# feng-li/dlsa

Hardware: AMD Instinct MI355X
Metric: rows/sec through X'WX kernel at p=500 (higher is better)
Workload: dtype f64

## Files before the change

### dlsa_amd/csrc/gram_cyclic.hip

```cpp
#include "common.h"
#ifndef DLSA_CYC_SPLIT
#define DLSA_CYC_SPLIT 1
#endif
#include <algorithm>
#ifndef DLSA_CYC_FLAGS
#define DLSA_CYC_FLAGS 0
#endif
#ifndef DLSA_CYC_PAIR
#define DLSA_CYC_PAIR 0
#endif
#ifndef DLSA_CYC_PRIO
#define DLSA_CYC_PRIO 0
#endif

namespace dlsa {

template <typename T>
void gram_reduce_launch(const T* partial, int nslab, int PP, int p, T* H, int64_t ldh, int accumulate, hipStream_t stream);

constexpr int CYC_NT = 31;
constexpr int CYC_C0 = 16 * CYC_NT;
constexpr int CYC_KC = 8;
constexpr int CYC_NST = 4;
constexpr int CYC_LDP = 528;
constexpr int CYC_BUF = CYC_KC * CYC_LDP + CYC_KC;
constexpr int CYC_GROUP = 4;
constexpr int CYC_PP = 512;
constexpr int CYC_MIN_P = 481, CYC_MAX_P = 508;
constexpr int64_t CYC_MIN_ROWS = 65536;

struct CycArgs {
    const double* X;
    const double* w;
    double* partial;
    int64_t ldx, n, rows_per_slab;
    int p;
    int nslab;
    unsigned long long* clk;
};

#include "gram_cyclic_asm.inc"

template <int T, int TEND, typename F>
__device__ __forceinline__ void cyc_for_tiles(F&& fn) {
    if constexpr (T < TEND) {
        double v[4];
        cyc_tile_read<T>(v);
        fn(T, v);
        cyc_for_tiles<T + 1, TEND>(fn);
    }
}

template <int K, int KEND, typename F>
__device__ __forceinline__ void cyc_for_tails(F&& fn) {
    if constexpr (K < KEND) {
        fn(K, cyc_tail_read<K>());
        cyc_for_tails<K + 1, KEND>(fn);
    }
}

template <bool HASW, int G>
__global__ __launch_bounds__(512, 2) void gram_cyclic_kernel(CycArgs a) {
    typedef __attribute__((address_space(3))) void* lds_ptr_t;
    constexpr int KC = CYC_KC, LDP = CYC_LDP, BUF = CYC_BUF, GA = G > 0 ? G : 1;
    constexpr int RW = 2, NW = 8, NB = RW + 7;
    constexpr int PIECES = KC * 4 / NW;
    constexpr int PPR = PIECES / RW;
    constexpr int DMA_PER_CHUNK = PIECES + (HASW ? 1 : 0);
    static_assert(KC == 8 && PPR * RW == PIECES && CYC_NST == 4, "pipeline shape");
    static_assert((BUF + 4 * LDP) * 8 + 128 < 65536, "stage parity + k-step offsets must fit a ds_read immediate");
    extern __shared__ __attribute__((aligned(16))) double lds[];
    const int tid = threadIdx.x, lane = tid & 63;
    const int wave = __builtin_amdgcn_readfirstlane(tid >> 6);
    const bool probe = blockIdx.x == 0 && wave == 0;
    const unsigned long long t_begin = probe ? __builtin_readcyclecounter() : 0ull;
    const int b = blockIdx.x, xcd = b % kNumXCD, jb = b / kNumXCD;
    const int slab = (jb / CYC_GROUP) * kNumXCD + xcd, member = jb % CYC_GROUP;
    const int rb = member * 4 + (wave & 3), db = wave >> 2;
    const int i0 = RW * rb, d0 = 8 * db;
    const bool two_rows = rb != 15;
    const bool tails = G > 0 && db == 0;

    const int64_t rbeg = (int64_t)slab * a.rows_per_slab;
    const int64_t rend = min(rbeg + a.rows_per_slab, a.n);
    const int64_t nrows = rend > rbeg ? rend - rbeg : 0;
    const int nchunks = (int)((nrows + KC - 1) / KC);

    const unsigned xbytes = nrows > 0 ? (unsigned)(((nrows - 1) * a.ldx + a.p) * 8) : 0u;
    __amdgpu_buffer_rsrc_t rsrcX = __builtin_amdgcn_make_buffer_rsrc((void*)(a.X + rbeg * a.ldx), 0, (int)xbytes, 0x00020000);
    __amdgpu_buffer_rsrc_t rsrcW =
        __builtin_amdgcn_make_buffer_rsrc((void*)(HASW ? a.w + rbeg : a.X), 0, HASW ? (int)(nrows * 8) : 0, 0x00020000);

    auto dma_piece = [&](int chunk, int buf, int pc) {
        const int id = pc * NW + wave, row = id >> 2, q = id & 3;
        const int soff = (int)((((int64_t)chunk * KC + row) * a.ldx + 128 * q) * 8);
        __builtin_amdgcn_raw_ptr_buffer_load_lds(rsrcX, (lds_ptr_t)(lds + buf * BUF + row * LDP + 128 * q), 16, lane * 16, soff, 0, 0);
    };
    auto dma_w = [&](int chunk, int buf) {
        if (HASW && lane < KC / 2)
            __builtin_amdgcn_raw_ptr_buffer_load_lds(rsrcW, (lds_ptr_t)(lds + buf * BUF + KC * LDP), 16, lane * 16, chunk * KC * 8, 0, 0);
    };

    cyc_acc_zero<128>();
    if constexpr (G > 0) cyc_tail_zero<2 * RW * G>();

#pragma unroll
    for (int ch = 0; ch < (DLSA_CYC_PAIR ? 2 : 3); ++ch) {
#pragma unroll
        for (int pc = 0; pc < PIECES; ++pc) dma_piece(ch, ch, pc);
        dma_w(ch, ch);
    }
#if DLSA_CYC_FLAGS
    unsigned long long* const flagL = reinterpret_cast<unsigned long long*>(lds + CYC_NST * BUF);
    unsigned long long* const flagD = flagL + 4;
    if (tid < 8) flagL[tid] = 0ull;
    __syncthreads();
    auto tag_of = [](int c) { return (unsigned)(((c >> 2) + 1) & 255); };
    auto post = [&](unsigned long long* f, int stage, int c) {
        if (lane == 0) reinterpret_cast<volatile unsigned char*>(f + stage)[wave] = (unsigned char)tag_of(c);
    };
    auto await = [&](unsigned long long* f, int stage, int c) {
        const unsigned long long want = 0x0101010101010101ull * tag_of(c);
        while (__builtin_amdgcn_readfirstlane((int)(*reinterpret_cast<volatile unsigned long long*>(f + stage) != want)))
            __builtin_amdgcn_s_sleep(1);
    };
    asm volatile("s_waitcnt vmcnt(%0)" ::"n"(2 * DMA_PER_CHUNK) : "memory");
    post(flagL, 0, 0);
    await(flagL, 0, 0);
#else
    asm volatile("s_waitcnt vmcnt(%0)" ::"n"(DLSA_CYC_PAIR ? 0 : 2 * DMA_PER_CHUNK) : "memory");
    asm volatile("s_barrier" ::: "memory");
#endif

    const int lane_part = ((lane >> 4) * LDP + (lane & 15)) * 8;
    int adA[2][RW], adB[2][NB], adT[2], adW[2];
#pragma unroll
    for (int sp = 0; sp < 2; ++sp) {
        const int sb = sp * 2 * BUF * 8;
        adA[sp][0] = sb + lane_part + 128 * i0;
        adA[sp][1] = sb + lane_part + 128 * (i0 + 1);
#pragma unroll
        for (int j = 0; j < NB; ++j) adB[sp][j] = sb + lane_part + 128 * ((i0 + d0 + j) % CYC_NT);
        adT[sp] = sb + ((lane >> 4) * LDP + CYC_C0 + (lane & 3)) * 8;
        adW[sp] = sb + (KC * LDP + (lane >> 4)) * 8;
    }
    const char* ldsb = (const char*)lds;
    struct Frag { double fa[RW], fb[NB], bt[GA], wv; };
    auto ld = [&](int addr, int imm) { return *(const double*)(ldsb + addr + imm); };
    auto load_frags = [&](int ST, int ks, Frag& f) {
        const int sp = ST >> 1, imm = ((ST & 1) * BUF + ks * 4 * LDP) * 8;
#pragma unroll
        for (int r = 0; r < RW; ++r) f.fa[r] = ld(adA[sp][r], imm);
#pragma unroll
        for (int j = 0; j < NB; ++j) f.fb[j] = ld(adB[sp][j], imm);
        if (tails) {
#pragma unroll
            for (int g = 0; g < G; ++g) f.bt[g] = ld(adT[sp], imm + 32 * g);
        }
        f.wv = HASW ? ld(adW[sp], ((ST & 1) * BUF + ks * 4) * 8) : 1.0;
    };
    auto kstep = [&](const Frag& f, int chunk_dma, int buf_dma, bool issue) {
        double aw[RW];
#pragma unroll
        for (int r = 0; r < RW; ++r) aw[r] = HASW ? f.fa[r] * f.wv : f.fa[r];
        cyc_row<0>(aw[0], f.fb[0], f.fb[1], f.fb[2], f.fb[3], f.fb[4], f.fb[5], f.fb[6], f.fb[7]);
        if (issue) {
#pragma unroll
            for (int k = 0; k < PPR; ++k) dma_piece(chunk_dma, buf_dma, k);
        }
        if (G > 0 || two_rows)
            cyc_row<1>(aw[1], f.fb[1], f.fb[2], f.fb[3], f.fb[4], f.fb[5], f.fb[6], f.fb[7], f.fb[8]);
        if (issue) {
#pragma unroll
            for (int k = 0; k < PPR; ++k) dma_piece(chunk_dma, buf_dma, PPR + k);
            dma_w(chunk_dma, buf_dma);
        }
        if constexpr (G > 0) {
            if (tails) cyc_tail_a<RW, G>(aw, f.bt);
        }
    };

    Frag fr0, fr1;
    load_frags(0, 0, fr0);
    if (DLSA_CYC_PRIO == 1 && db) __builtin_amdgcn_s_setprio(1);
    if (DLSA_CYC_PRIO == 2 && !db) __builtin_amdgcn_s_setprio(1);
#if DLSA_CYC_FLAGS
    for (int c4 = 0; c4 < nchunks; c4 += 4) {
#pragma unroll
        for (int u = 0; u < 4; ++u) {
            const int c = c4 + u;
            load_frags(u, 1, fr1);
            if (c > 0) post(flagD, (u + 3) & 3, c - 1);
            __builtin_amdgcn_sched_barrier(0);
            {
                double aw[RW];
#pragma unroll
                for (int r = 0; r < RW; ++r) aw[r] = HASW ? fr0.fa[r] * fr0.wv : fr0.fa[r];
                cyc_row<0>(aw[0], fr0.fb[0], fr0.fb[1], fr0.fb[2], fr0.fb[3], fr0.fb[4], fr0.fb[5], fr0.fb[6], fr0.fb[7]);
                __builtin_amdgcn_sched_barrier(0);
                asm volatile("s_waitcnt vmcnt(%0)" ::"n"(DMA_PER_CHUNK) : "memory");
                post(flagL, (u + 1) & 3, c + 1);
                __builtin_amdgcn_sched_barrier(0);
                if (G > 0 || two_rows)
                    cyc_row<1>(aw[1], fr0.fb[1], fr0.fb[2], fr0.fb[3], fr0.fb[4], fr0.fb[5], fr0.fb[6], fr0.fb[7], fr0.fb[8]);
                if constexpr (G > 0) {
                    if (tails) cyc_tail_a<RW, G>(aw, fr0.bt);
                }
                __builtin_amdgcn_sched_barrier(0);
            }
            await(flagL, (u + 1) & 3, c + 1);
            load_frags((u + 1) & 3, 0, fr0);
            __builtin_amdgcn_sched_barrier(0);
            if (c > 0) await(flagD, (u + 3) & 3, c - 1);
            __builtin_amdgcn_sched_barrier(0);
            kstep(fr1, c + 3, (u + 3) & 3, true);
            __builtin_amdgcn_sched_barrier(0);
        }
    }
#elif DLSA_CYC_PAIR
    for (int c4 = 0; c4 < nchunks; c4 += 4) {
#pragma unroll
        for (int u = 0; u < 4; u += 2) {
            const int c = c4 + u;
            load_frags(u, 1, fr1);
            __builtin_amdgcn_sched_barrier(0);
            kstep(fr0, c + 2, (u + 2) & 3, true);
            __builtin_amdgcn_sched_barrier(0);
            load_frags(u + 1, 0, fr0);
            __builtin_amdgcn_sched_barrier(0);
            kstep(fr1, c + 3, (u + 3) & 3, true);
            __builtin_amdgcn_sched_barrier(0);
            load_frags(u + 1, 1, fr1);
            __builtin_amdgcn_sched_barrier(0);
            kstep(fr0, 0, 0, false);
            __builtin_amdgcn_sched_barrier(0);
            {
                double aw[RW];
#pragma unroll
                for (int r = 0; r < RW; ++r) aw[r] = HASW ? fr1.fa[r] * fr1.wv : fr1.fa[r];
                cyc_row<0>(aw[0], fr1.fb[0], fr1.fb[1], fr1.fb[2], fr1.fb[3], fr1.fb[4], fr1.fb[5], fr1.fb[6], fr1.fb[7]);
                __builtin_amdgcn_sched_barrier(0);
                if (db) {
                    asm volatile("s_waitcnt vmcnt(0)" ::: "memory");
                    asm volatile("s_barrier" ::: "memory");
                }
                if (G > 0 || two_rows)
                    cyc_row<1>(aw[1], fr1.fb[1], fr1.fb[2], fr1.fb[3], fr1.fb[4], fr1.fb[5], fr1.fb[6], fr1.fb[7], fr1.fb[8]);
                if constexpr (G > 0) {
                    if (tails) cyc_tail_a<RW, G>(aw, fr1.bt);
                }
                __builtin_amdgcn_sched_barrier(0);
                if (!db) {
                    asm volatile("s_waitcnt vmcnt(0)" ::: "memory");
                    asm volatile("s_barrier" ::: "memory");
                }
            }
            load_frags((u + 2) & 3, 0, fr0);
            __builtin_amdgcn_sched_barrier(0);
        }
    }
#else
    for (int c4 = 0; c4 < nchunks; c4 += 4) {
#pragma unroll
        for (int u = 0; u < 4; ++u) {
            load_frags(u, 1, fr1);
            __builtin_amdgcn_sched_barrier(0);
#if DLSA_CYC_SPLIT
            {
                double aw[RW];
#pragma unroll
                for (int r = 0; r < RW; ++r) aw[r] = HASW ? fr0.fa[r] * fr0.wv : fr0.fa[r];
                cyc_row<0>(aw[0], fr0.fb[0], fr0.fb[1], fr0.fb[2], fr0.fb[3], fr0.fb[4], fr0.fb[5], fr0.fb[6], fr0.fb[7]);
                __builtin_amdgcn_sched_barrier(0);
                if (db) {
                    asm volatile("s_waitcnt vmcnt(%0)" ::"n"(DMA_PER_CHUNK) : "memory");
                    asm volatile("s_barrier" ::: "memory");
                }
                if (G > 0 || two_rows)
                    cyc_row<1>(aw[1], fr0.fb[1], fr0.fb[2], fr0.fb[3], fr0.fb[4], fr0.fb[5], fr0.fb[6], fr0.fb[7], fr0.fb[8]);
                if constexpr (G > 0) {
                    if (tails) cyc_tail_a<RW, G>(aw, fr0.bt);
                }
                __builtin_amdgcn_sched_barrier(0);
                if (!db) {
                    asm volatile("s_waitcnt vmcnt(%0)" ::"n"(DMA_PER_CHUNK) : "memory");
                    asm volatile("s_barrier" ::: "memory");
                }
            }
#else
            kstep(fr0, 0, 0, false);
            __builtin_amdgcn_sched_barrier(0);
            asm volatile("s_waitcnt vmcnt(%0)" ::"n"(DMA_PER_CHUNK) : "memory");
            asm volatile("s_barrier" ::: "memory");
#endif
            load_frags((u + 1) & 3, 0, fr0);
            __builtin_amdgcn_sched_barrier(0);
            kstep(fr1, c4 + u + 3, (u + 3) & 3, true);
            __builtin_amdgcn_sched_barrier(0);
        }
    }
#endif
    asm volatile("s_waitcnt vmcnt(0)" ::: "memory");
    asm volatile("s_nop 15\n\ts_nop 15" ::: "memory");

    double* __restrict__ P = a.partial + (int64_t)slab * CYC_PP * CYC_PP;
    const int nt_rows = two_rows ? 2 : 1;
    cyc_for_tiles<0, 8 * RW>([&](int k, double (&v)[4]) {
        const int r = k >> 3, cdist = k & 7;
        if (r < nt_rows) {
            const int it = i0 + r, jt = (it + d0 + cdist) % CYC_NT;
#pragma unroll
            for (int q = 0; q < 4; ++q) {
                const int rr = 16 * it + 4 * q + (lane >> 4), cc = 16 * jt + (lane & 15);
                if (jt >= it) P[(int64_t)rr * CYC_PP + cc] = v[q];
                else P[(int64_t)cc * CYC_PP + rr] = v[q];
            }
        }
    });
    if constexpr (G > 0) {
        if (tails) cyc_for_tails<0, RW * G>([&](int idx, double v) {
            const int s = idx / G, g = idx - s * G;
            const int row = 16 * (i0 + s) + 4 * ((lane & 15) >> 2) + (lane >> 4), col = CYC_C0 + 4 * g + (lane & 3);
            P[(int64_t)row * CYC_PP + col] = v;
        });
    }
    if (probe && lane == 0) *a.clk = __builtin_readcyclecounter() - t_begin;
}

static int cyc_slabs(int64_t n, int64_t& rows_per_slab) {
    int64_t ns = kNumCU / CYC_GROUP;
    while (ns > kNumXCD && n / ns < 4 * CYC_KC) ns -= kNumXCD;
    rows_per_slab = ((n + ns - 1) / ns + CYC_KC - 1) / CYC_KC * CYC_KC;
    return (int)ns;
}

bool gram_cyclic_shape_ok(int64_t n, int p) { return p >= CYC_MIN_P && p <= CYC_MAX_P && n >= CYC_MIN_ROWS; }

bool gram_cyclic_eligible(const double* X, int64_t ldx, const double* w, int64_t n, int p) {
    if (!gram_cyclic_shape_ok(n, p)) return false;
    if (gram_dbg_env() & 8) return false;
    int64_t rps;
    cyc_slabs(n, rps);
    return ldx % 2 == 0 && ((uintptr_t)X % 16) == 0 && (!w || ((uintptr_t)w % 16) == 0) &&
           (double)(rps + 8 * CYC_KC) * (double)ldx * 8.0 < 2.0e9;
}

size_t gram_cyclic_ws_bytes(int64_t n, int p) {
    int64_t rps;
    return align_up((size_t)cyc_slabs(n, rps) * CYC_PP * CYC_PP * 8, 256) + kGramProbeBytes;
}

int gram_cyclic_f64(const double* X, int64_t ldx, const double* w, int64_t n, int p, double* H, int64_t ldh,
                    int accumulate, void* ws, size_t ws_bytes, hipStream_t stream) {
    CycArgs a;
    a.X = X; a.w = w; a.partial = (double*)ws; a.ldx = ldx; a.n = n;
    a.p = p + (p & 1);
    a.nslab = cyc_slabs(n, a.rows_per_slab);
    const size_t need = align_up((size_t)a.nslab * CYC_PP * CYC_PP * 8, 256) + kGramProbeBytes;
    a.clk = (unsigned long long*)((char*)ws + need - kGramProbeBytes);
    if (!ws || ws_bytes < need || ((uintptr_t)ws & 255)) {
        set_error("gram: workspace %zu bytes needed (256-aligned), got %zu", need, ws_bytes);
        return DLSA_ERR_WORKSPACE;
    }
    const int g = a.p <= CYC_C0 ? 0 : (a.p - CYC_C0 + 3) / 4;
    const size_t shm = (size_t)CYC_NST * CYC_BUF * 8 + (DLSA_CYC_FLAGS ? 64 : 0);
    const int blocks = a.nslab * CYC_GROUP;
#define DLSA_LAUNCH_CYC(HW, GV) do { \
        DLSA_HIP_CHECK(hipFuncSetAttribute(reinterpret_cast<const void*>(gram_cyclic_kernel<HW, GV>), \
                                           hipFuncAttributeMaxDynamicSharedMemorySize, (int)shm)); \
        hipLaunchKernelGGL((gram_cyclic_kernel<HW, GV>), dim3(blocks), dim3(512), shm, stream, a); } while (0)
#define DLSA_LAUNCH_CYC_G(HW) do { switch (g) { \
        case 0: DLSA_LAUNCH_CYC(HW, 0); break; case 1: DLSA_LAUNCH_CYC(HW, 1); break; \
        case 2: DLSA_LAUNCH_CYC(HW, 2); break; default: DLSA_LAUNCH_CYC(HW, 3); break; } } while (0)
    if (w) DLSA_LAUNCH_CYC_G(true);
    else DLSA_LAUNCH_CYC_G(false);
    note_gram_kernel(a.clk, stream, "gram_cyclic_kernel<%s,%d>", w ? "true" : "false", g > 3 ? 3 : g);
#undef DLSA_LAUNCH_CYC_G
#undef DLSA_LAUNCH_CYC
    DLSA_HIP_CHECK(hipGetLastError());
    gram_reduce_launch<double>((const double*)ws, a.nslab, CYC_PP, p, H, ldh, accumulate, stream);
    DLSA_HIP_CHECK(hipGetLastError());
    return DLSA_OK;
}

}
```

### dlsa_amd/csrc/gram_cyclic_asm.inc

```
template <int NREG> __device__ __forceinline__ void cyc_acc_zero();
template <> __device__ __forceinline__ void cyc_acc_zero<128>() {
    asm volatile("v_accvgpr_write_b32 a0, 0\n\tv_accvgpr_write_b32 a1, 0\n\tv_accvgpr_write_b32 a2, 0\n\tv_accvgpr_write_b32 a3, 0\n\tv_accvgpr_write_b32 a4, 0\n\tv_accvgpr_write_b32 a5, 0\n\tv_accvgpr_write_b32 a6, 0\n\tv_accvgpr_write_b32 a7, 0\n\tv_accvgpr_write_b32 a8, 0\n\tv_accvgpr_write_b32 a9, 0\n\tv_accvgpr_write_b32 a10, 0\n\tv_accvgpr_write_b32 a11, 0\n\tv_accvgpr_write_b32 a12, 0\n\tv_accvgpr_write_b32 a13, 0\n\tv_accvgpr_write_b32 a14, 0\n\tv_accvgpr_write_b32 a15, 0\n\tv_accvgpr_write_b32 a16, 0\n\tv_accvgpr_write_b32 a17, 0\n\tv_accvgpr_write_b32 a18, 0\n\tv_accvgpr_write_b32 a19, 0\n\tv_accvgpr_write_b32 a20, 0\n\tv_accvgpr_write_b32 a21, 0\n\tv_accvgpr_write_b32 a22, 0\n\tv_accvgpr_write_b32 a23, 0\n\tv_accvgpr_write_b32 a24, 0\n\tv_accvgpr_write_b32 a25, 0\n\tv_accvgpr_write_b32 a26, 0\n\tv_accvgpr_write_b32 a27, 0\n\tv_accvgpr_write_b32 a28, 0\n\tv_accvgpr_write_b32 a29, 0\n\tv_accvgpr_write_b32 a30, 0\n\tv_accvgpr_write_b32 a31, 0\n\tv_accvgpr_write_b32 a32, 0\n\tv_accvgpr_write_b32 a33, 0\n\tv_accvgpr_write_b32 a34, 0\n\tv_accvgpr_write_b32 a35, 0\n\tv_accvgpr_write_b32 a36, 0\n\tv_accvgpr_write_b32 a37, 0\n\tv_accvgpr_write_b32 a38, 0\n\tv_accvgpr_write_b32 a39, 0\n\tv_accvgpr_write_b32 a40, 0\n\tv_accvgpr_write_b32 a41, 0\n\tv_accvgpr_write_b32 a42, 0\n\tv_accvgpr_write_b32 a43, 0\n\tv_accvgpr_write_b32 a44, 0\n\tv_accvgpr_write_b32 a45, 0\n\tv_accvgpr_write_b32 a46, 0\n\tv_accvgpr_write_b32 a47, 0\n\tv_accvgpr_write_b32 a48, 0\n\tv_accvgpr_write_b32 a49, 0\n\tv_accvgpr_write_b32 a50, 0\n\tv_accvgpr_write_b32 a51, 0\n\tv_accvgpr_write_b32 a52, 0\n\tv_accvgpr_write_b32 a53, 0\n\tv_accvgpr_write_b32 a54, 0\n\tv_accvgpr_write_b32 a55, 0\n\tv_accvgpr_write_b32 a56, 0\n\tv_accvgpr_write_b32 a57, 0\n\tv_accvgpr_write_b32 a58, 0\n\tv_accvgpr_write_b32 a59, 0\n\tv_accvgpr_write_b32 a60, 0\n\tv_accvgpr_write_b32 a61, 0\n\tv_accvgpr_write_b32 a62, 0\n\tv_accvgpr_write_b32 a63, 0\n\tv_accvgpr_write_b32 a64, 0\n\tv_accvgpr_write_b32 a65, 0\n\tv_accvgpr_write_b32 a66, 0\n\tv_accvgpr_write_b32 a67, 0\n\tv_accvgpr_write_b32 a68, 0\n\tv_accvgpr_write_b32 a69, 0\n\tv_accvgpr_write_b32 a70, 0\n\tv_accvgpr_write_b32 a71, 0\n\tv_accvgpr_write_b32 a72, 0\n\tv_accvgpr_write_b32 a73, 0\n\tv_accvgpr_write_b32 a74, 0\n\tv_accvgpr_write_b32 a75, 0\n\tv_accvgpr_write_b32 a76, 0\n\tv_accvgpr_write_b32 a77, 0\n\tv_accvgpr_write_b32 a78, 0\n\tv_accvgpr_write_b32 a79, 0\n\tv_accvgpr_write_b32 a80, 0\n\tv_accvgpr_write_b32 a81, 0\n\tv_accvgpr_write_b32 a82, 0\n\tv_accvgpr_write_b32 a83, 0\n\tv_accvgpr_write_b32 a84, 0\n\tv_accvgpr_write_b32 a85, 0\n\tv_accvgpr_write_b32 a86, 0\n\tv_accvgpr_write_b32 a87, 0\n\tv_accvgpr_write_b32 a88, 0\n\tv_accvgpr_write_b32 a89, 0\n\tv_accvgpr_write_b32 a90, 0\n\tv_accvgpr_write_b32 a91, 0\n\tv_accvgpr_write_b32 a92, 0\n\tv_accvgpr_write_b32 a93, 0\n\tv_accvgpr_write_b32 a94, 0\n\tv_accvgpr_write_b32 a95, 0\n\tv_accvgpr_write_b32 a96, 0\n\tv_accvgpr_write_b32 a97, 0\n\tv_accvgpr_write_b32 a98, 0\n\tv_accvgpr_write_b32 a99, 0\n\tv_accvgpr_write_b32 a100, 0\n\tv_accvgpr_write_b32 a101, 0\n\tv_accvgpr_write_b32 a102, 0\n\tv_accvgpr_write_b32 a103, 0\n\tv_accvgpr_write_b32 a104, 0\n\tv_accvgpr_write_b32 a105, 0\n\tv_accvgpr_write_b32 a106, 0\n\tv_accvgpr_write_b32 a107, 0\n\tv_accvgpr_write_b32 a108, 0\n\tv_accvgpr_write_b32 a109, 0\n\tv_accvgpr_write_b32 a110, 0\n\tv_accvgpr_write_b32 a111, 0\n\tv_accvgpr_write_b32 a112, 0\n\tv_accvgpr_write_b32 a113, 0\n\tv_accvgpr_write_b32 a114, 0\n\tv_accvgpr_write_b32 a115, 0\n\tv_accvgpr_write_b32 a116, 0\n\tv_accvgpr_write_b32 a117, 0\n\tv_accvgpr_write_b32 a118, 0\n\tv_accvgpr_write_b32 a119, 0\n\tv_accvgpr_write_b32 a120, 0\n\tv_accvgpr_write_b32 a121, 0\n\tv_accvgpr_write_b32 a122, 0\n\tv_accvgpr_write_b32 a123, 0\n\tv_accvgpr_write_b32 a124, 0\n\tv_accvgpr_write_b32 a125, 0\n\tv_accvgpr_write_b32 a126, 0\n\tv_accvgpr_write_b32 a127, 0" ::: "a0", "a1", "a2", "a3", "a4", "a5", "a6", "a7", "a8", "a9", "a10", "a11", "a12", "a13", "a14", "a15", "a16", "a17", "a18", "a19", "a20", "a21", "a22", "a23", "a24", "a25", "a26", "a27", "a28", "a29", "a30", "a31", "a32", "a33", "a34", "a35", "a36", "a37", "a38", "a39", "a40", "a41", "a42", "a43", "a44", "a45", "a46", "a47", "a48", "a49", "a50", "a51", "a52", "a53", "a54", "a55", "a56", "a57", "a58", "a59", "a60", "a61", "a62", "a63", "a64", "a65", "a66", "a67", "a68", "a69", "a70", "a71", "a72", "a73", "a74", "a75", "a76", "a77", "a78", "a79", "a80", "a81", "a82", "a83", "a84", "a85", "a86", "a87", "a88", "a89", "a90", "a91", "a92", "a93", "a94", "a95", "a96", "a97", "a98", "a99", "a100", "a101", "a102", "a103", "a104", "a105", "a106", "a107", "a108", "a109", "a110", "a111", "a112", "a113", "a114", "a115", "a116", "a117", "a118", "a119", "a120", "a121", "a122", "a123", "a124", "a125", "a126", "a127");
}
template <> __device__ __forceinline__ void cyc_acc_zero<256>() {
    asm volatile("v_accvgpr_write_b32 a0, 0\n\tv_accvgpr_write_b32 a1, 0\n\tv_accvgpr_write_b32 a2, 0\n\tv_accvgpr_write_b32 a3, 0\n\tv_accvgpr_write_b32 a4, 0\n\tv_accvgpr_write_b32 a5, 0\n\tv_accvgpr_write_b32 a6, 0\n\tv_accvgpr_write_b32 a7, 0\n\tv_accvgpr_write_b32 a8, 0\n\tv_accvgpr_write_b32 a9, 0\n\tv_accvgpr_write_b32 a10, 0\n\tv_accvgpr_write_b32 a11, 0\n\tv_accvgpr_write_b32 a12, 0\n\tv_accvgpr_write_b32 a13, 0\n\tv_accvgpr_write_b32 a14, 0\n\tv_accvgpr_write_b32 a15, 0\n\tv_accvgpr_write_b32 a16, 0\n\tv_accvgpr_write_b32 a17, 0\n\tv_accvgpr_write_b32 a18, 0\n\tv_accvgpr_write_b32 a19, 0\n\tv_accvgpr_write_b32 a20, 0\n\tv_accvgpr_write_b32 a21, 0\n\tv_accvgpr_write_b32 a22, 0\n\tv_accvgpr_write_b32 a23, 0\n\tv_accvgpr_write_b32 a24, 0\n\tv_accvgpr_write_b32 a25, 0\n\tv_accvgpr_write_b32 a26, 0\n\tv_accvgpr_write_b32 a27, 0\n\tv_accvgpr_write_b32 a28, 0\n\tv_accvgpr_write_b32 a29, 0\n\tv_accvgpr_write_b32 a30, 0\n\tv_accvgpr_write_b32 a31, 0\n\tv_accvgpr_write_b32 a32, 0\n\tv_accvgpr_write_b32 a33, 0\n\tv_accvgpr_write_b32 a34, 0\n\tv_accvgpr_write_b32 a35, 0\n\tv_accvgpr_write_b32 a36, 0\n\tv_accvgpr_write_b32 a37, 0\n\tv_accvgpr_write_b32 a38, 0\n\tv_accvgpr_write_b32 a39, 0\n\tv_accvgpr_write_b32 a40, 0\n\tv_accvgpr_write_b32 a41, 0\n\tv_accvgpr_write_b32 a42, 0\n\tv_accvgpr_write_b32 a43, 0\n\tv_accvgpr_write_b32 a44, 0\n\tv_accvgpr_write_b32 a45, 0\n\tv_accvgpr_write_b32 a46, 0\n\tv_accvgpr_write_b32 a47, 0\n\tv_accvgpr_write_b32 a48, 0\n\tv_accvgpr_write_b32 a49, 0\n\tv_accvgpr_write_b32 a50, 0\n\tv_accvgpr_write_b32 a51, 0\n\tv_accvgpr_write_b32 a52, 0\n\tv_accvgpr_write_b32 a53, 0\n\tv_accvgpr_write_b32 a54, 0\n\tv_accvgpr_write_b32 a55, 0\n\tv_accvgpr_write_b32 a56, 0\n\tv_accvgpr_write_b32 a57, 0\n\tv_accvgpr_write_b32 a58, 0\n\tv_accvgpr_write_b32 a59, 0\n\tv_accvgpr_write_b32 a60, 0\n\tv_accvgpr_write_b32 a61, 0\n\tv_accvgpr_write_b32 a62, 0\n\tv_accvgpr_write_b32 a63, 0\n\tv_accvgpr_write_b32 a64, 0\n\tv_accvgpr_write_b32 a65, 0\n\tv_accvgpr_write_b32 a66, 0\n\tv_accvgpr_write_b32 a67, 0\n\tv_accvgpr_write_b32 a68, 0\n\tv_accvgpr_write_b32 a69, 0\n\tv_accvgpr_write_b32 a70, 0\n\tv_accvgpr_write_b32 a71, 0\n\tv_accvgpr_write_b32 a72, 0\n\tv_accvgpr_write_b32 a73, 0\n\tv_accvgpr_write_b32 a74, 0\n\tv_accvgpr_write_b32 a75, 0\n\tv_accvgpr_write_b32 a76, 0\n\tv_accvgpr_write_b32 a77, 0\n\tv_accvgpr_write_b32 a78, 0\n\tv_accvgpr_write_b32 a79, 0\n\tv_accvgpr_write_b32 a80, 0\n\tv_accvgpr_write_b32 a81, 0\n\tv_accvgpr_write_b32 a82, 0\n\tv_accvgpr_write_b32 a83, 0\n\tv_accvgpr_write_b32 a84, 0\n\tv_accvgpr_write_b32 a85, 0\n\tv_accvgpr_write_b32 a86, 0\n\tv_accvgpr_write_b32 a87, 0\n\tv_accvgpr_write_b32 a88, 0\n\tv_accvgpr_write_b32 a89, 0\n\tv_accvgpr_write_b32 a90, 0\n\tv_accvgpr_write_b32 a91, 0\n\tv_accvgpr_write_b32 a92, 0\n\tv_accvgpr_write_b32 a93, 0\n\tv_accvgpr_write_b32 a94, 0\n\tv_accvgpr_write_b32 a95, 0\n\tv_accvgpr_write_b32 a96, 0\n\tv_accvgpr_write_b32 a97, 0\n\tv_accvgpr_write_b32 a98, 0\n\tv_accvgpr_write_b32 a99, 0\n\tv_accvgpr_write_b32 a100, 0\n\tv_accvgpr_write_b32 a101, 0\n\tv_accvgpr_write_b32 a102, 0\n\tv_accvgpr_write_b32 a103, 0\n\tv_accvgpr_write_b32 a104, 0\n\tv_accvgpr_write_b32 a105, 0\n\tv_accvgpr_write_b32 a106, 0\n\tv_accvgpr_write_b32 a107, 0\n\tv_accvgpr_write_b32 a108, 0\n\tv_accvgpr_write_b32 a109, 0\n\tv_accvgpr_write_b32 a110, 0\n\tv_accvgpr_write_b32 a111, 0\n\tv_accvgpr_write_b32 a112, 0\n\tv_accvgpr_write_b32 a113, 0\n\tv_accvgpr_write_b32 a114, 0\n\tv_accvgpr_write_b32 a115, 0\n\tv_accvgpr_write_b32 a116, 0\n\tv_accvgpr_write_b32 a117, 0\n\tv_accvgpr_write_b32 a118, 0\n\tv_accvgpr_write_b32 a119, 0\n\tv_accvgpr_write_b32 a120, 0\n\tv_accvgpr_write_b32 a121, 0\n\tv_accvgpr_write_b32 a122, 0\n\tv_accvgpr_write_b32 a123, 0\n\tv_accvgpr_write_b32 a124, 0\n\tv_accvgpr_write_b32 a125, 0\n\tv_accvgpr_write_b32 a126, 0\n\tv_accvgpr_write_b32 a127, 0\n\tv_accvgpr_write_b32 a128, 0\n\tv_accvgpr_write_b32 a129, 0\n\tv_accvgpr_write_b32 a130, 0\n\tv_accvgpr_write_b32 a131, 0\n\tv_accvgpr_write_b32 a132, 0\n\tv_accvgpr_write_b32 a133, 0\n\tv_accvgpr_write_b32 a134, 0\n\tv_accvgpr_write_b32 a135, 0\n\tv_accvgpr_write_b32 a136, 0\n\tv_accvgpr_write_b32 a137, 0\n\tv_accvgpr_write_b32 a138, 0\n\tv_accvgpr_write_b32 a139, 0\n\tv_accvgpr_write_b32 a140, 0\n\tv_accvgpr_write_b32 a141, 0\n\tv_accvgpr_write_b32 a142, 0\n\tv_accvgpr_write_b32 a143, 0\n\tv_accvgpr_write_b32 a144, 0\n\tv_accvgpr_write_b32 a145, 0\n\tv_accvgpr_write_b32 a146, 0\n\tv_accvgpr_write_b32 a147, 0\n\tv_accvgpr_write_b32 a148, 0\n\tv_accvgpr_write_b32 a149, 0\n\tv_accvgpr_write_b32 a150, 0\n\tv_accvgpr_write_b32 a151, 0\n\tv_accvgpr_write_b32 a152, 0\n\tv_accvgpr_write_b32 a153, 0\n\tv_accvgpr_write_b32 a154, 0\n\tv_accvgpr_write_b32 a155, 0\n\tv_accvgpr_write_b32 a156, 0\n\tv_accvgpr_write_b32 a157, 0\n\tv_accvgpr_write_b32 a158, 0\n\tv_accvgpr_write_b32 a159, 0\n\tv_accvgpr_write_b32 a160, 0\n\tv_accvgpr_write_b32 a161, 0\n\tv_accvgpr_write_b32 a162, 0\n\tv_accvgpr_write_b32 a163, 0\n\tv_accvgpr_write_b32 a164, 0\n\tv_accvgpr_write_b32 a165, 0\n\tv_accvgpr_write_b32 a166, 0\n\tv_accvgpr_write_b32 a167, 0\n\tv_accvgpr_write_b32 a168, 0\n\tv_accvgpr_write_b32 a169, 0\n\tv_accvgpr_write_b32 a170, 0\n\tv_accvgpr_write_b32 a171, 0\n\tv_accvgpr_write_b32 a172, 0\n\tv_accvgpr_write_b32 a173, 0\n\tv_accvgpr_write_b32 a174, 0\n\tv_accvgpr_write_b32 a175, 0\n\tv_accvgpr_write_b32 a176, 0\n\tv_accvgpr_write_b32 a177, 0\n\tv_accvgpr_write_b32 a178, 0\n\tv_accvgpr_write_b32 a179, 0\n\tv_accvgpr_write_b32 a180, 0\n\tv_accvgpr_write_b32 a181, 0\n\tv_accvgpr_write_b32 a182, 0\n\tv_accvgpr_write_b32 a183, 0\n\tv_accvgpr_write_b32 a184, 0\n\tv_accvgpr_write_b32 a185, 0\n\tv_accvgpr_write_b32 a186, 0\n\tv_accvgpr_write_b32 a187, 0\n\tv_accvgpr_write_b32 a188, 0\n\tv_accvgpr_write_b32 a189, 0\n\tv_accvgpr_write_b32 a190, 0\n\tv_accvgpr_write_b32 a191, 0\n\tv_accvgpr_write_b32 a192, 0\n\tv_accvgpr_write_b32 a193, 0\n\tv_accvgpr_write_b32 a194, 0\n\tv_accvgpr_write_b32 a195, 0\n\tv_accvgpr_write_b32 a196, 0\n\tv_accvgpr_write_b32 a197, 0\n\tv_accvgpr_write_b32 a198, 0\n\tv_accvgpr_write_b32 a199, 0\n\tv_accvgpr_write_b32 a200, 0\n\tv_accvgpr_write_b32 a201, 0\n\tv_accvgpr_write_b32 a202, 0\n\tv_accvgpr_write_b32 a203, 0\n\tv_accvgpr_write_b32 a204, 0\n\tv_accvgpr_write_b32 a205, 0\n\tv_accvgpr_write_b32 a206, 0\n\tv_accvgpr_write_b32 a207, 0\n\tv_accvgpr_write_b32 a208, 0\n\tv_accvgpr_write_b32 a209, 0\n\tv_accvgpr_write_b32 a210, 0\n\tv_accvgpr_write_b32 a211, 0\n\tv_accvgpr_write_b32 a212, 0\n\tv_accvgpr_write_b32 a213, 0\n\tv_accvgpr_write_b32 a214, 0\n\tv_accvgpr_write_b32 a215, 0\n\tv_accvgpr_write_b32 a216, 0\n\tv_accvgpr_write_b32 a217, 0\n\tv_accvgpr_write_b32 a218, 0\n\tv_accvgpr_write_b32 a219, 0\n\tv_accvgpr_write_b32 a220, 0\n\tv_accvgpr_write_b32 a221, 0\n\tv_accvgpr_write_b32 a222, 0\n\tv_accvgpr_write_b32 a223, 0\n\tv_accvgpr_write_b32 a224, 0\n\tv_accvgpr_write_b32 a225, 0\n\tv_accvgpr_write_b32 a226, 0\n\tv_accvgpr_write_b32 a227, 0\n\tv_accvgpr_write_b32 a228, 0\n\tv_accvgpr_write_b32 a229, 0\n\tv_accvgpr_write_b32 a230, 0\n\tv_accvgpr_write_b32 a231, 0\n\tv_accvgpr_write_b32 a232, 0\n\tv_accvgpr_write_b32 a233, 0\n\tv_accvgpr_write_b32 a234, 0\n\tv_accvgpr_write_b32 a235, 0\n\tv_accvgpr_write_b32 a236, 0\n\tv_accvgpr_write_b32 a237, 0\n\tv_accvgpr_write_b32 a238, 0\n\tv_accvgpr_write_b32 a239, 0\n\tv_accvgpr_write_b32 a240, 0\n\tv_accvgpr_write_b32 a241, 0\n\tv_accvgpr_write_b32 a242, 0\n\tv_accvgpr_write_b32 a243, 0\n\tv_accvgpr_write_b32 a244, 0\n\tv_accvgpr_write_b32 a245, 0\n\tv_accvgpr_write_b32 a246, 0\n\tv_accvgpr_write_b32 a247, 0\n\tv_accvgpr_write_b32 a248, 0\n\tv_accvgpr_write_b32 a249, 0\n\tv_accvgpr_write_b32 a250, 0\n\tv_accvgpr_write_b32 a251, 0\n\tv_accvgpr_write_b32 a252, 0\n\tv_accvgpr_write_b32 a253, 0\n\tv_accvgpr_write_b32 a254, 0\n\tv_accvgpr_write_b32 a255, 0" ::: "a0", "a1", "a2", "a3", "a4", "a5", "a6", "a7", "a8", "a9", "a10", "a11", "a12", "a13", "a14", "a15", "a16", "a17", "a18", "a19", "a20", "a21", "a22", "a23", "a24", "a25", "a26", "a27", "a28", "a29", "a30", "a31", "a32", "a33", "a34", "a35", "a36", "a37", "a38", "a39", "a40", "a41", "a42", "a43", "a44", "a45", "a46", "a47", "a48", "a49", "a50", "a51", "a52", "a53", "a54", "a55", "a56", "a57", "a58", "a59", "a60", "a61", "a62", "a63", "a64", "a65", "a66", "a67", "a68", "a69", "a70", "a71", "a72", "a73", "a74", "a75", "a76", "a77", "a78", "a79", "a80", "a81", "a82", "a83", "a84", "a85", "a86", "a87", "a88", "a89", "a90", "a91", "a92", "a93", "a94", "a95", "a96", "a97", "a98", "a99", "a100", "a101", "a102", "a103", "a104", "a105", "a106", "a107", "a108", "a109", "a110", "a111", "a112", "a113", "a114", "a115", "a116", "a117", "a118", "a119", "a120", "a121", "a122", "a123", "a124", "a125", "a126", "a127", "a128", "a129", "a130", "a131", "a132", "a133", "a134", "a135", "a136", "a137", "a138", "a139", "a140", "a141", "a142", "a143", "a144", "a145", "a146", "a147", "a148", "a149", "a150", "a151", "a152", "a153", "a154", "a155", "a156", "a157", "a158", "a159", "a160", "a161", "a162", "a163", "a164", "a165", "a166", "a167", "a168", "a169", "a170", "a171", "a172", "a173", "a174", "a175", "a176", "a177", "a178", "a179", "a180", "a181", "a182", "a183", "a184", "a185", "a186", "a187", "a188", "a189", "a190", "a191", "a192", "a193", "a194", "a195", "a196", "a197", "a198", "a199", "a200", "a201", "a202", "a203", "a204", "a205", "a206", "a207", "a208", "a209", "a210", "a211", "a212", "a213", "a214", "a215", "a216", "a217", "a218", "a219", "a220", "a221", "a222", "a223", "a224", "a225", "a226", "a227", "a228", "a229", "a230", "a231", "a232", "a233", "a234", "a235", "a236", "a237", "a238", "a239", "a240", "a241", "a242", "a243", "a244", "a245", "a246", "a247", "a248", "a249", "a250", "a251", "a252", "a253", "a254", "a255");
}
template <int R> __device__ __forceinline__ void cyc_row(double a, double b0, double b1, double b2, double b3, double b4, double b5, double b6, double b7);
template <> __device__ __forceinline__ void cyc_row<0>(double a, double b0, double b1, double b2, double b3, double b4, double b5, double b6, double b7) {
    asm volatile("s_nop 1\n\tv_mfma_f64_16x16x4_f64 a[0:7], %0, %1, a[0:7]\n\tv_mfma_f64_16x16x4_f64 a[8:15], %0, %2, a[8:15]\n\tv_mfma_f64_16x16x4_f64 a[16:23], %0, %3, a[16:23]\n\tv_mfma_f64_16x16x4_f64 a[24:31], %0, %4, a[24:31]\n\tv_mfma_f64_16x16x4_f64 a[32:39], %0, %5, a[32:39]\n\tv_mfma_f64_16x16x4_f64 a[40:47], %0, %6, a[40:47]\n\tv_mfma_f64_16x16x4_f64 a[48:55], %0, %7, a[48:55]\n\tv_mfma_f64_16x16x4_f64 a[56:63], %0, %8, a[56:63]"
                 :: "v"(a), "v"(b0), "v"(b1), "v"(b2), "v"(b3), "v"(b4), "v"(b5), "v"(b6), "v"(b7)
                 : "a0", "a1", "a2", "a3", "a4", "a5", "a6", "a7", "a8", "a9", "a10", "a11", "a12", "a13", "a14", "a15", "a16", "a17", "a18", "a19", "a20", "a21", "a22", "a23", "a24", "a25", "a26", "a27", "a28", "a29", "a30", "a31", "a32", "a33", "a34", "a35", "a36", "a37", "a38", "a39", "a40", "a41", "a42", "a43", "a44", "a45", "a46", "a47", "a48", "a49", "a50", "a51", "a52", "a53", "a54", "a55", "a56", "a57", "a58", "a59", "a60", "a61", "a62", "a63");
}
template <> __device__ __forceinline__ void cyc_row<1>(double a, double b0, double b1, double b2, double b3, double b4, double b5, double b6, double b7) {
    asm volatile("s_nop 1\n\tv_mfma_f64_16x16x4_f64 a[64:71], %0, %1, a[64:71]\n\tv_mfma_f64_16x16x4_f64 a[72:79], %0, %2, a[72:79]\n\tv_mfma_f64_16x16x4_f64 a[80:87], %0, %3, a[80:87]\n\tv_mfma_f64_16x16x4_f64 a[88:95], %0, %4, a[88:95]\n\tv_mfma_f64_16x16x4_f64 a[96:103], %0, %5, a[96:103]\n\tv_mfma_f64_16x16x4_f64 a[104:111], %0, %6, a[104:111]\n\tv_mfma_f64_16x16x4_f64 a[112:119], %0, %7, a[112:119]\n\tv_mfma_f64_16x16x4_f64 a[120:127], %0, %8, a[120:127]"
                 :: "v"(a), "v"(b0), "v"(b1), "v"(b2), "v"(b3), "v"(b4), "v"(b5), "v"(b6), "v"(b7)
                 : "a64", "a65", "a66", "a67", "a68", "a69", "a70", "a71", "a72", "a73", "a74", "a75", "a76", "a77", "a78", "a79", "a80", "a81", "a82", "a83", "a84", "a85", "a86", "a87", "a88", "a89", "a90", "a91", "a92", "a93", "a94", "a95", "a96", "a97", "a98", "a99", "a100", "a101", "a102", "a103", "a104", "a105", "a106", "a107", "a108", "a109", "a110", "a111", "a112", "a113", "a114", "a115", "a116", "a117", "a118", "a119", "a120", "a121", "a122", "a123", "a124", "a125", "a126", "a127");
}
template <> __device__ __forceinline__ void cyc_row<2>(double a, double b0, double b1, double b2, double b3, double b4, double b5, double b6, double b7) {
    asm volatile("s_nop 1\n\tv_mfma_f64_16x16x4_f64 a[128:135], %0, %1, a[128:135]\n\tv_mfma_f64_16x16x4_f64 a[136:143], %0, %2, a[136:143]\n\tv_mfma_f64_16x16x4_f64 a[144:151], %0, %3, a[144:151]\n\tv_mfma_f64_16x16x4_f64 a[152:159], %0, %4, a[152:159]\n\tv_mfma_f64_16x16x4_f64 a[160:167], %0, %5, a[160:167]\n\tv_mfma_f64_16x16x4_f64 a[168:175], %0, %6, a[168:175]\n\tv_mfma_f64_16x16x4_f64 a[176:183], %0, %7, a[176:183]\n\tv_mfma_f64_16x16x4_f64 a[184:191], %0, %8, a[184:191]"
                 :: "v"(a), "v"(b0), "v"(b1), "v"(b2), "v"(b3), "v"(b4), "v"(b5), "v"(b6), "v"(b7)
                 : "a128", "a129", "a130", "a131", "a132", "a133", "a134", "a135", "a136", "a137", "a138", "a139", "a140", "a141", "a142", "a143", "a144", "a145", "a146", "a147", "a148", "a149", "a150", "a151", "a152", "a153", "a154", "a155", "a156", "a157", "a158", "a159", "a160", "a161", "a162", "a163", "a164", "a165", "a166", "a167", "a168", "a169", "a170", "a171", "a172", "a173", "a174", "a175", "a176", "a177", "a178", "a179", "a180", "a181", "a182", "a183", "a184", "a185", "a186", "a187", "a188", "a189", "a190", "a191");
}
template <> __device__ __forceinline__ void cyc_row<3>(double a, double b0, double b1, double b2, double b3, double b4, double b5, double b6, double b7) {
    asm volatile("s_nop 1\n\tv_mfma_f64_16x16x4_f64 a[192:199], %0, %1, a[192:199]\n\tv_mfma_f64_16x16x4_f64 a[200:207], %0, %2, a[200:207]\n\tv_mfma_f64_16x16x4_f64 a[208:215], %0, %3, a[208:215]\n\tv_mfma_f64_16x16x4_f64 a[216:223], %0, %4, a[216:223]\n\tv_mfma_f64_16x16x4_f64 a[224:231], %0, %5, a[224:231]\n\tv_mfma_f64_16x16x4_f64 a[232:239], %0, %6, a[232:239]\n\tv_mfma_f64_16x16x4_f64 a[240:247], %0, %7, a[240:247]\n\tv_mfma_f64_16x16x4_f64 a[248:255], %0, %8, a[248:255]"
                 :: "v"(a), "v"(b0), "v"(b1), "v"(b2), "v"(b3), "v"(b4), "v"(b5), "v"(b6), "v"(b7)
                 : "a192", "a193", "a194", "a195", "a196", "a197", "a198", "a199", "a200", "a201", "a202", "a203", "a204", "a205", "a206", "a207", "a208", "a209", "a210", "a211", "a212", "a213", "a214", "a215", "a216", "a217", "a218", "a219", "a220", "a221", "a222", "a223", "a224", "a225", "a226", "a227", "a228", "a229", "a230", "a231", "a232", "a233", "a234", "a235", "a236", "a237", "a238", "a239", "a240", "a241", "a242", "a243", "a244", "a245", "a246", "a247", "a248", "a249", "a250", "a251", "a252", "a253", "a254", "a255");
}
template <int TS, int G> __device__ __forceinline__ void cyc_tail_a(const double (&at)[TS], const double (&bt)[G > 0 ? G : 1]);
template <int N> __device__ __forceinline__ void cyc_tail_zero();
template <> __device__ __forceinline__ void cyc_tail_zero<4>() {
    asm volatile("v_accvgpr_write_b32 a128, 0\n\tv_accvgpr_write_b32 a129, 0\n\tv_accvgpr_write_b32 a130, 0\n\tv_accvgpr_write_b32 a131, 0" ::: "a128", "a129", "a130", "a131");
}
template <> __device__ __forceinline__ void cyc_tail_zero<8>() {
    asm volatile("v_accvgpr_write_b32 a128, 0\n\tv_accvgpr_write_b32 a129, 0\n\tv_accvgpr_write_b32 a130, 0\n\tv_accvgpr_write_b32 a131, 0\n\tv_accvgpr_write_b32 a132, 0\n\tv_accvgpr_write_b32 a133, 0\n\tv_accvgpr_write_b32 a134, 0\n\tv_accvgpr_write_b32 a135, 0" ::: "a128", "a129", "a130", "a131", "a132", "a133", "a134", "a135");
}
template <> __device__ __forceinline__ void cyc_tail_zero<12>() {
    asm volatile("v_accvgpr_write_b32 a128, 0\n\tv_accvgpr_write_b32 a129, 0\n\tv_accvgpr_write_b32 a130, 0\n\tv_accvgpr_write_b32 a131, 0\n\tv_accvgpr_write_b32 a132, 0\n\tv_accvgpr_write_b32 a133, 0\n\tv_accvgpr_write_b32 a134, 0\n\tv_accvgpr_write_b32 a135, 0\n\tv_accvgpr_write_b32 a136, 0\n\tv_accvgpr_write_b32 a137, 0\n\tv_accvgpr_write_b32 a138, 0\n\tv_accvgpr_write_b32 a139, 0" ::: "a128", "a129", "a130", "a131", "a132", "a133", "a134", "a135", "a136", "a137", "a138", "a139");
}
template <> __device__ __forceinline__ void cyc_tail_a<2, 0>(const double (&)[2], const double (&)[1]) {}
template <> __device__ __forceinline__ void cyc_tail_a<2, 1>(const double (&at)[2], const double (&bt)[1]) {
    asm volatile("v_mfma_f64_4x4x4_4b_f64 a[128:129], %0, %2, a[128:129]\n\tv_mfma_f64_4x4x4_4b_f64 a[130:131], %1, %2, a[130:131]"
                 :: "v"(at[0]), "v"(at[1]), "v"(bt[0])
                 : "a128", "a129", "a130", "a131");
}
template <> __device__ __forceinline__ void cyc_tail_a<2, 2>(const double (&at)[2], const double (&bt)[2]) {
    asm volatile("v_mfma_f64_4x4x4_4b_f64 a[128:129], %0, %2, a[128:129]\n\tv_mfma_f64_4x4x4_4b_f64 a[130:131], %0, %3, a[130:131]\n\tv_mfma_f64_4x4x4_4b_f64 a[132:133], %1, %2, a[132:133]\n\tv_mfma_f64_4x4x4_4b_f64 a[134:135], %1, %3, a[134:135]"
                 :: "v"(at[0]), "v"(at[1]), "v"(bt[0]), "v"(bt[1])
                 : "a128", "a129", "a130", "a131", "a132", "a133", "a134", "a135");
}
template <> __device__ __forceinline__ void cyc_tail_a<2, 3>(const double (&at)[2], const double (&bt)[3]) {
    asm volatile("v_mfma_f64_4x4x4_4b_f64 a[128:129], %0, %2, a[128:129]\n\tv_mfma_f64_4x4x4_4b_f64 a[130:131], %0, %3, a[130:131]\n\tv_mfma_f64_4x4x4_4b_f64 a[132:133], %0, %4, a[132:133]\n\tv_mfma_f64_4x4x4_4b_f64 a[134:135], %1, %2, a[134:135]\n\tv_mfma_f64_4x4x4_4b_f64 a[136:137], %1, %3, a[136:137]\n\tv_mfma_f64_4x4x4_4b_f64 a[138:139], %1, %4, a[138:139]"
                 :: "v"(at[0]), "v"(at[1]), "v"(bt[0]), "v"(bt[1]), "v"(bt[2])
                 : "a128", "a129", "a130", "a131", "a132", "a133", "a134", "a135", "a136", "a137", "a138", "a139");
}
template <int IDX> __device__ __forceinline__ double cyc_tail_read() {
    int lo, hi;
    if constexpr (IDX == 0) asm volatile("v_accvgpr_read_b32 %0, a128\n\tv_accvgpr_read_b32 %1, a129" : "=v"(lo), "=v"(hi));
    else if constexpr (IDX == 1) asm volatile("v_accvgpr_read_b32 %0, a130\n\tv_accvgpr_read_b32 %1, a131" : "=v"(lo), "=v"(hi));
    else if constexpr (IDX == 2) asm volatile("v_accvgpr_read_b32 %0, a132\n\tv_accvgpr_read_b32 %1, a133" : "=v"(lo), "=v"(hi));
    else if constexpr (IDX == 3) asm volatile("v_accvgpr_read_b32 %0, a134\n\tv_accvgpr_read_b32 %1, a135" : "=v"(lo), "=v"(hi));
    else if constexpr (IDX == 4) asm volatile("v_accvgpr_read_b32 %0, a136\n\tv_accvgpr_read_b32 %1, a137" : "=v"(lo), "=v"(hi));
    else if constexpr (IDX == 5) asm volatile("v_accvgpr_read_b32 %0, a138\n\tv_accvgpr_read_b32 %1, a139" : "=v"(lo), "=v"(hi));
    return __hiloint2double(hi, lo);
}
template <int T> __device__ __forceinline__ void cyc_tile_read(double (&v)[4]) {
    int w0, w1, w2, w3, w4, w5, w6, w7;
    if constexpr (T == 0) asm volatile("v_accvgpr_read_b32 %0, a0\n\tv_accvgpr_read_b32 %1, a1\n\tv_accvgpr_read_b32 %2, a2\n\tv_accvgpr_read_b32 %3, a3\n\tv_accvgpr_read_b32 %4, a4\n\tv_accvgpr_read_b32 %5, a5\n\tv_accvgpr_read_b32 %6, a6\n\tv_accvgpr_read_b32 %7, a7" : "=v"(w0), "=v"(w1), "=v"(w2), "=v"(w3), "=v"(w4), "=v"(w5), "=v"(w6), "=v"(w7));
    else if constexpr (T == 1) asm volatile("v_accvgpr_read_b32 %0, a8\n\tv_accvgpr_read_b32 %1, a9\n\tv_accvgpr_read_b32 %2, a10\n\tv_accvgpr_read_b32 %3, a11\n\tv_accvgpr_read_b32 %4, a12\n\tv_accvgpr_read_b32 %5, a13\n\tv_accvgpr_read_b32 %6, a14\n\tv_accvgpr_read_b32 %7, a15" : "=v"(w0), "=v"(w1), "=v"(w2), "=v"(w3), "=v"(w4), "=v"(w5), "=v"(w6), "=v"(w7));
    else if constexpr (T == 2) asm volatile("v_accvgpr_read_b32 %0, a16\n\tv_accvgpr_read_b32 %1, a17\n\tv_accvgpr_read_b32 %2, a18\n\tv_accvgpr_read_b32 %3, a19\n\tv_accvgpr_read_b32 %4, a20\n\tv_accvgpr_read_b32 %5, a21\n\tv_accvgpr_read_b32 %6, a22\n\tv_accvgpr_read_b32 %7, a23" : "=v"(w0), "=v"(w1), "=v"(w2), "=v"(w3), "=v"(w4), "=v"(w5), "=v"(w6), "=v"(w7));
    else if constexpr (T == 3) asm volatile("v_accvgpr_read_b32 %0, a24\n\tv_accvgpr_read_b32 %1, a25\n\tv_accvgpr_read_b32 %2, a26\n\tv_accvgpr_read_b32 %3, a27\n\tv_accvgpr_read_b32 %4, a28\n\tv_accvgpr_read_b32 %5, a29\n\tv_accvgpr_read_b32 %6, a30\n\tv_accvgpr_read_b32 %7, a31" : "=v"(w0), "=v"(w1), "=v"(w2), "=v"(w3), "=v"(w4), "=v"(w5), "=v"(w6), "=v"(w7));
    else if constexpr (T == 4) asm volatile("v_accvgpr_read_b32 %0, a32\n\tv_accvgpr_read_b32 %1, a33\n\tv_accvgpr_read_b32 %2, a34\n\tv_accvgpr_read_b32 %3, a35\n\tv_accvgpr_read_b32 %4, a36\n\tv_accvgpr_read_b32 %5, a37\n\tv_accvgpr_read_b32 %6, a38\n\tv_accvgpr_read_b32 %7, a39" : "=v"(w0), "=v"(w1), "=v"(w2), "=v"(w3), "=v"(w4), "=v"(w5), "=v"(w6), "=v"(w7));
    else if constexpr (T == 5) asm volatile("v_accvgpr_read_b32 %0, a40\n\tv_accvgpr_read_b32 %1, a41\n\tv_accvgpr_read_b32 %2, a42\n\tv_accvgpr_read_b32 %3, a43\n\tv_accvgpr_read_b32 %4, a44\n\tv_accvgpr_read_b32 %5, a45\n\tv_accvgpr_read_b32 %6, a46\n\tv_accvgpr_read_b32 %7, a47" : "=v"(w0), "=v"(w1), "=v"(w2), "=v"(w3), "=v"(w4), "=v"(w5), "=v"(w6), "=v"(w7));
    else if constexpr (T == 6) asm volatile("v_accvgpr_read_b32 %0, a48\n\tv_accvgpr_read_b32 %1, a49\n\tv_accvgpr_read_b32 %2, a50\n\tv_accvgpr_read_b32 %3, a51\n\tv_accvgpr_read_b32 %4, a52\n\tv_accvgpr_read_b32 %5, a53\n\tv_accvgpr_read_b32 %6, a54\n\tv_accvgpr_read_b32 %7, a55" : "=v"(w0), "=v"(w1), "=v"(w2), "=v"(w3), "=v"(w4), "=v"(w5), "=v"(w6), "=v"(w7));
    else if constexpr (T == 7) asm volatile("v_accvgpr_read_b32 %0, a56\n\tv_accvgpr_read_b32 %1, a57\n\tv_accvgpr_read_b32 %2, a58\n\tv_accvgpr_read_b32 %3, a59\n\tv_accvgpr_read_b32 %4, a60\n\tv_accvgpr_read_b32 %5, a61\n\tv_accvgpr_read_b32 %6, a62\n\tv_accvgpr_read_b32 %7, a63" : "=v"(w0), "=v"(w1), "=v"(w2), "=v"(w3), "=v"(w4), "=v"(w5), "=v"(w6), "=v"(w7));
    else if constexpr (T == 8) asm volatile("v_accvgpr_read_b32 %0, a64\n\tv_accvgpr_read_b32 %1, a65\n\tv_accvgpr_read_b32 %2, a66\n\tv_accvgpr_read_b32 %3, a67\n\tv_accvgpr_read_b32 %4, a68\n\tv_accvgpr_read_b32 %5, a69\n\tv_accvgpr_read_b32 %6, a70\n\tv_accvgpr_read_b32 %7, a71" : "=v"(w0), "=v"(w1), "=v"(w2), "=v"(w3), "=v"(w4), "=v"(w5), "=v"(w6), "=v"(w7));
    else if constexpr (T == 9) asm volatile("v_accvgpr_read_b32 %0, a72\n\tv_accvgpr_read_b32 %1, a73\n\tv_accvgpr_read_b32 %2, a74\n\tv_accvgpr_read_b32 %3, a75\n\tv_accvgpr_read_b32 %4, a76\n\tv_accvgpr_read_b32 %5, a77\n\tv_accvgpr_read_b32 %6, a78\n\tv_accvgpr_read_b32 %7, a79" : "=v"(w0), "=v"(w1), "=v"(w2), "=v"(w3), "=v"(w4), "=v"(w5), "=v"(w6), "=v"(w7));
    else if constexpr (T == 10) asm volatile("v_accvgpr_read_b32 %0, a80\n\tv_accvgpr_read_b32 %1, a81\n\tv_accvgpr_read_b32 %2, a82\n\tv_accvgpr_read_b32 %3, a83\n\tv_accvgpr_read_b32 %4, a84\n\tv_accvgpr_read_b32 %5, a85\n\tv_accvgpr_read_b32 %6, a86\n\tv_accvgpr_read_b32 %7, a87" : "=v"(w0), "=v"(w1), "=v"(w2), "=v"(w3), "=v"(w4), "=v"(w5), "=v"(w6), "=v"(w7));
    else if constexpr (T == 11) asm volatile("v_accvgpr_read_b32 %0, a88\n\tv_accvgpr_read_b32 %1, a89\n\tv_accvgpr_read_b32 %2, a90\n\tv_accvgpr_read_b32 %3, a91\n\tv_accvgpr_read_b32 %4, a92\n\tv_accvgpr_read_b32 %5, a93\n\tv_accvgpr_read_b32 %6, a94\n\tv_accvgpr_read_b32 %7, a95" : "=v"(w0), "=v"(w1), "=v"(w2), "=v"(w3), "=v"(w4), "=v"(w5), "=v"(w6), "=v"(w7));
    else if constexpr (T == 12) asm volatile("v_accvgpr_read_b32 %0, a96\n\tv_accvgpr_read_b32 %1, a97\n\tv_accvgpr_read_b32 %2, a98\n\tv_accvgpr_read_b32 %3, a99\n\tv_accvgpr_read_b32 %4, a100\n\tv_accvgpr_read_b32 %5, a101\n\tv_accvgpr_read_b32 %6, a102\n\tv_accvgpr_read_b32 %7, a103" : "=v"(w0), "=v"(w1), "=v"(w2), "=v"(w3), "=v"(w4), "=v"(w5), "=v"(w6), "=v"(w7));
    else if constexpr (T == 13) asm volatile("v_accvgpr_read_b32 %0, a104\n\tv_accvgpr_read_b32 %1, a105\n\tv_accvgpr_read_b32 %2, a106\n\tv_accvgpr_read_b32 %3, a107\n\tv_accvgpr_read_b32 %4, a108\n\tv_accvgpr_read_b32 %5, a109\n\tv_accvgpr_read_b32 %6, a110\n\tv_accvgpr_read_b32 %7, a111" : "=v"(w0), "=v"(w1), "=v"(w2), "=v"(w3), "=v"(w4), "=v"(w5), "=v"(w6), "=v"(w7));
    else if constexpr (T == 14) asm volatile("v_accvgpr_read_b32 %0, a112\n\tv_accvgpr_read_b32 %1, a113\n\tv_accvgpr_read_b32 %2, a114\n\tv_accvgpr_read_b32 %3, a115\n\tv_accvgpr_read_b32 %4, a116\n\tv_accvgpr_read_b32 %5, a117\n\tv_accvgpr_read_b32 %6, a118\n\tv_accvgpr_read_b32 %7, a119" : "=v"(w0), "=v"(w1), "=v"(w2), "=v"(w3), "=v"(w4), "=v"(w5), "=v"(w6), "=v"(w7));
    else if constexpr (T == 15) asm volatile("v_accvgpr_read_b32 %0, a120\n\tv_accvgpr_read_b32 %1, a121\n\tv_accvgpr_read_b32 %2, a122\n\tv_accvgpr_read_b32 %3, a123\n\tv_accvgpr_read_b32 %4, a124\n\tv_accvgpr_read_b32 %5, a125\n\tv_accvgpr_read_b32 %6, a126\n\tv_accvgpr_read_b32 %7, a127" : "=v"(w0), "=v"(w1), "=v"(w2), "=v"(w3), "=v"(w4), "=v"(w5), "=v"(w6), "=v"(w7));
    else if constexpr (T == 16) asm volatile("v_accvgpr_read_b32 %0, a128\n\tv_accvgpr_read_b32 %1, a129\n\tv_accvgpr_read_b32 %2, a130\n\tv_accvgpr_read_b32 %3, a131\n\tv_accvgpr_read_b32 %4, a132\n\tv_accvgpr_read_b32 %5, a133\n\tv_accvgpr_read_b32 %6, a134\n\tv_accvgpr_read_b32 %7, a135" : "=v"(w0), "=v"(w1), "=v"(w2), "=v"(w3), "=v"(w4), "=v"(w5), "=v"(w6), "=v"(w7));
    else if constexpr (T == 17) asm volatile("v_accvgpr_read_b32 %0, a136\n\tv_accvgpr_read_b32 %1, a137\n\tv_accvgpr_read_b32 %2, a138\n\tv_accvgpr_read_b32 %3, a139\n\tv_accvgpr_read_b32 %4, a140\n\tv_accvgpr_read_b32 %5, a141\n\tv_accvgpr_read_b32 %6, a142\n\tv_accvgpr_read_b32 %7, a143" : "=v"(w0), "=v"(w1), "=v"(w2), "=v"(w3), "=v"(w4), "=v"(w5), "=v"(w6), "=v"(w7));
    else if constexpr (T == 18) asm volatile("v_accvgpr_read_b32 %0, a144\n\tv_accvgpr_read_b32 %1, a145\n\tv_accvgpr_read_b32 %2, a146\n\tv_accvgpr_read_b32 %3, a147\n\tv_accvgpr_read_b32 %4, a148\n\tv_accvgpr_read_b32 %5, a149\n\tv_accvgpr_read_b32 %6, a150\n\tv_accvgpr_read_b32 %7, a151" : "=v"(w0), "=v"(w1), "=v"(w2), "=v"(w3), "=v"(w4), "=v"(w5), "=v"(w6), "=v"(w7));
    else if constexpr (T == 19) asm volatile("v_accvgpr_read_b32 %0, a152\n\tv_accvgpr_read_b32 %1, a153\n\tv_accvgpr_read_b32 %2, a154\n\tv_accvgpr_read_b32 %3, a155\n\tv_accvgpr_read_b32 %4, a156\n\tv_accvgpr_read_b32 %5, a157\n\tv_accvgpr_read_b32 %6, a158\n\tv_accvgpr_read_b32 %7, a159" : "=v"(w0), "=v"(w1), "=v"(w2), "=v"(w3), "=v"(w4), "=v"(w5), "=v"(w6), "=v"(w7));
    else if constexpr (T == 20) asm volatile("v_accvgpr_read_b32 %0, a160\n\tv_accvgpr_read_b32 %1, a161\n\tv_accvgpr_read_b32 %2, a162\n\tv_accvgpr_read_b32 %3, a163\n\tv_accvgpr_read_b32 %4, a164\n\tv_accvgpr_read_b32 %5, a165\n\tv_accvgpr_read_b32 %6, a166\n\tv_accvgpr_read_b32 %7, a167" : "=v"(w0), "=v"(w1), "=v"(w2), "=v"(w3), "=v"(w4), "=v"(w5), "=v"(w6), "=v"(w7));
    else if constexpr (T == 21) asm volatile("v_accvgpr_read_b32 %0, a168\n\tv_accvgpr_read_b32 %1, a169\n\tv_accvgpr_read_b32 %2, a170\n\tv_accvgpr_read_b32 %3, a171\n\tv_accvgpr_read_b32 %4, a172\n\tv_accvgpr_read_b32 %5, a173\n\tv_accvgpr_read_b32 %6, a174\n\tv_accvgpr_read_b32 %7, a175" : "=v"(w0), "=v"(w1), "=v"(w2), "=v"(w3), "=v"(w4), "=v"(w5), "=v"(w6), "=v"(w7));
    else if constexpr (T == 22) asm volatile("v_accvgpr_read_b32 %0, a176\n\tv_accvgpr_read_b32 %1, a177\n\tv_accvgpr_read_b32 %2, a178\n\tv_accvgpr_read_b32 %3, a179\n\tv_accvgpr_read_b32 %4, a180\n\tv_accvgpr_read_b32 %5, a181\n\tv_accvgpr_read_b32 %6, a182\n\tv_accvgpr_read_b32 %7, a183" : "=v"(w0), "=v"(w1), "=v"(w2), "=v"(w3), "=v"(w4), "=v"(w5), "=v"(w6), "=v"(w7));
    else if constexpr (T == 23) asm volatile("v_accvgpr_read_b32 %0, a184\n\tv_accvgpr_read_b32 %1, a185\n\tv_accvgpr_read_b32 %2, a186\n\tv_accvgpr_read_b32 %3, a187\n\tv_accvgpr_read_b32 %4, a188\n\tv_accvgpr_read_b32 %5, a189\n\tv_accvgpr_read_b32 %6, a190\n\tv_accvgpr_read_b32 %7, a191" : "=v"(w0), "=v"(w1), "=v"(w2), "=v"(w3), "=v"(w4), "=v"(w5), "=v"(w6), "=v"(w7));
    else if constexpr (T == 24) asm volatile("v_accvgpr_read_b32 %0, a192\n\tv_accvgpr_read_b32 %1, a193\n\tv_accvgpr_read_b32 %2, a194\n\tv_accvgpr_read_b32 %3, a195\n\tv_accvgpr_read_b32 %4, a196\n\tv_accvgpr_read_b32 %5, a197\n\tv_accvgpr_read_b32 %6, a198\n\tv_accvgpr_read_b32 %7, a199" : "=v"(w0), "=v"(w1), "=v"(w2), "=v"(w3), "=v"(w4), "=v"(w5), "=v"(w6), "=v"(w7));
    else if constexpr (T == 25) asm volatile("v_accvgpr_read_b32 %0, a200\n\tv_accvgpr_read_b32 %1, a201\n\tv_accvgpr_read_b32 %2, a202\n\tv_accvgpr_read_b32 %3, a203\n\tv_accvgpr_read_b32 %4, a204\n\tv_accvgpr_read_b32 %5, a205\n\tv_accvgpr_read_b32 %6, a206\n\tv_accvgpr_read_b32 %7, a207" : "=v"(w0), "=v"(w1), "=v"(w2), "=v"(w3), "=v"(w4), "=v"(w5), "=v"(w6), "=v"(w7));
    else if constexpr (T == 26) asm volatile("v_accvgpr_read_b32 %0, a208\n\tv_accvgpr_read_b32 %1, a209\n\tv_accvgpr_read_b32 %2, a210\n\tv_accvgpr_read_b32 %3, a211\n\tv_accvgpr_read_b32 %4, a212\n\tv_accvgpr_read_b32 %5, a213\n\tv_accvgpr_read_b32 %6, a214\n\tv_accvgpr_read_b32 %7, a215" : "=v"(w0), "=v"(w1), "=v"(w2), "=v"(w3), "=v"(w4), "=v"(w5), "=v"(w6), "=v"(w7));
    else if constexpr (T == 27) asm volatile("v_accvgpr_read_b32 %0, a216\n\tv_accvgpr_read_b32 %1, a217\n\tv_accvgpr_read_b32 %2, a218\n\tv_accvgpr_read_b32 %3, a219\n\tv_accvgpr_read_b32 %4, a220\n\tv_accvgpr_read_b32 %5, a221\n\tv_accvgpr_read_b32 %6, a222\n\tv_accvgpr_read_b32 %7, a223" : "=v"(w0), "=v"(w1), "=v"(w2), "=v"(w3), "=v"(w4), "=v"(w5), "=v"(w6), "=v"(w7));
    else if constexpr (T == 28) asm volatile("v_accvgpr_read_b32 %0, a224\n\tv_accvgpr_read_b32 %1, a225\n\tv_accvgpr_read_b32 %2, a226\n\tv_accvgpr_read_b32 %3, a227\n\tv_accvgpr_read_b32 %4, a228\n\tv_accvgpr_read_b32 %5, a229\n\tv_accvgpr_read_b32 %6, a230\n\tv_accvgpr_read_b32 %7, a231" : "=v"(w0), "=v"(w1), "=v"(w2), "=v"(w3), "=v"(w4), "=v"(w5), "=v"(w6), "=v"(w7));
    else if constexpr (T == 29) asm volatile("v_accvgpr_read_b32 %0, a232\n\tv_accvgpr_read_b32 %1, a233\n\tv_accvgpr_read_b32 %2, a234\n\tv_accvgpr_read_b32 %3, a235\n\tv_accvgpr_read_b32 %4, a236\n\tv_accvgpr_read_b32 %5, a237\n\tv_accvgpr_read_b32 %6, a238\n\tv_accvgpr_read_b32 %7, a239" : "=v"(w0), "=v"(w1), "=v"(w2), "=v"(w3), "=v"(w4), "=v"(w5), "=v"(w6), "=v"(w7));
    else if constexpr (T == 30) asm volatile("v_accvgpr_read_b32 %0, a240\n\tv_accvgpr_read_b32 %1, a241\n\tv_accvgpr_read_b32 %2, a242\n\tv_accvgpr_read_b32 %3, a243\n\tv_accvgpr_read_b32 %4, a244\n\tv_accvgpr_read_b32 %5, a245\n\tv_accvgpr_read_b32 %6, a246\n\tv_accvgpr_read_b32 %7, a247" : "=v"(w0), "=v"(w1), "=v"(w2), "=v"(w3), "=v"(w4), "=v"(w5), "=v"(w6), "=v"(w7));
    else if constexpr (T == 31) asm volatile("v_accvgpr_read_b32 %0, a248\n\tv_accvgpr_read_b32 %1, a249\n\tv_accvgpr_read_b32 %2, a250\n\tv_accvgpr_read_b32 %3, a251\n\tv_accvgpr_read_b32 %4, a252\n\tv_accvgpr_read_b32 %5, a253\n\tv_accvgpr_read_b32 %6, a254\n\tv_accvgpr_read_b32 %7, a255" : "=v"(w0), "=v"(w1), "=v"(w2), "=v"(w3), "=v"(w4), "=v"(w5), "=v"(w6), "=v"(w7));
    v[0] = __hiloint2double(w1, w0); v[1] = __hiloint2double(w3, w2);
    v[2] = __hiloint2double(w5, w4); v[3] = __hiloint2double(w7, w6);
}
```

Measured before the change: 273.1 million.

## Add one-row-per-wave cyclic Gram variant with 1024-thread blocks and staggered barriers

Result: faster. 275.8 million, median of 6 (+1.0%).

```diff
diff --git a/dlsa_amd/csrc/gram_cyclic.hip b/dlsa_amd/csrc/gram_cyclic.hip
--- a/dlsa_amd/csrc/gram_cyclic.hip
+++ b/dlsa_amd/csrc/gram_cyclic.hip
@@ -3,15 +3,6 @@
 #define DLSA_CYC_SPLIT 1
 #endif
 #include <algorithm>
-#ifndef DLSA_CYC_FLAGS
-#define DLSA_CYC_FLAGS 0
-#endif
-#ifndef DLSA_CYC_PAIR
-#define DLSA_CYC_PAIR 0
-#endif
-#ifndef DLSA_CYC_PRIO
-#define DLSA_CYC_PRIO 0
-#endif
 
 namespace dlsa {
 
@@ -29,6 +20,10 @@
 constexpr int CYC_MIN_P = 481, CYC_MAX_P = 508;
 constexpr int64_t CYC_MIN_ROWS = 65536;
 
+constexpr int cyc_rw(int ) { return 1; }
+
+constexpr int CYC_BAR_Q[4] = {2, 1, 2, 1};
+
 struct CycArgs {
     const double* X;
     const double* w;
@@ -51,23 +46,23 @@
     }
 }
 
-template <int K, int KEND, typename F>
+template <int TS, int K, int KEND, typename F>
 __device__ __forceinline__ void cyc_for_tails(F&& fn) {
     if constexpr (K < KEND) {
-        fn(K, cyc_tail_read<K>());
-        cyc_for_tails<K + 1, KEND>(fn);
-    }
-}
-
-template <bool HASW, int G>
-__global__ __launch_bounds__(512, 2) void gram_cyclic_kernel(CycArgs a) {
+        fn(K, cyc_tail_read<TS, K>());
+        cyc_for_tails<TS, K + 1, KEND>(fn);
+    }
+}
+
+template <bool HASW, int G, int RW>
+__device__ __forceinline__ void cyc_body(const CycArgs& a) {
     typedef __attribute__((address_space(3))) void* lds_ptr_t;
     constexpr int KC = CYC_KC, LDP = CYC_LDP, BUF = CYC_BUF, GA = G > 0 ? G : 1;
-    constexpr int RW = 2, NW = 8, NB = RW + 7;
+    constexpr int NW = 16 / RW, NB = RW + 7;
     constexpr int PIECES = KC * 4 / NW;
-    constexpr int PPR = PIECES / RW;
+    constexpr int PPR = RW == 2 ? PIECES / RW : PIECES;
     constexpr int DMA_PER_CHUNK = PIECES + (HASW ? 1 : 0);
-    static_assert(KC == 8 && PPR * RW == PIECES && CYC_NST == 4, "pipeline shape");
+    static_assert((RW == 1 || RW == 2) && KC == 8 && CYC_NST == 4, "pipeline shape");
     static_assert((BUF + 4 * LDP) * 8 + 128 < 65536, "stage parity + k-step offsets must fit a ds_read immediate");
     extern __shared__ __attribute__((aligned(16))) double lds[];
     const int tid = threadIdx.x, lane = tid & 63;
@@ -76,9 +71,10 @@
     const unsigned long long t_begin = probe ? __builtin_readcyclecounter() : 0ull;
     const int b = blockIdx.x, xcd = b % kNumXCD, jb = b / kNumXCD;
     const int slab = (jb / CYC_GROUP) * kNumXCD + xcd, member = jb % CYC_GROUP;
-    const int rb = member * 4 + (wave & 3), db = wave >> 2;
-    const int i0 = RW * rb, d0 = 8 * db;
-    const bool two_rows = rb != 15;
+    const int rb = member * 4 + (wave & 3), slot = wave >> 2;
+    const int i0 = RW == 2 ? 2 * rb : 2 * rb + (slot & 1), db = RW == 2 ? slot : slot >> 1;
+    const int d0 = 8 * db;
+    const bool full_rows = i0 + RW - 1 != CYC_NT;
     const bool tails = G > 0 && db == 0;
 
     const int64_t rbeg = (int64_t)slab * a.rows_per_slab;
@@ -101,48 +97,37 @@
             __builtin_amdgcn_raw_ptr_buffer_load_lds(rsrcW, (lds_ptr_t)(lds + buf * BUF + KC * LDP), 16, lane * 16, chunk * KC * 8, 0, 0);
     };
 
-    cyc_acc_zero<128>();
-    if constexpr (G > 0) cyc_tail_zero<2 * RW * G>();
-
-#pragma unroll
-    for (int ch = 0; ch < (DLSA_CYC_PAIR ? 2 : 3); ++ch) {
+    cyc_acc_zero<64 * RW>();
+    if constexpr (G > 0) cyc_tail_zero<RW, G>();
+
+#pragma unroll
+    for (int ch = 0; ch < 3; ++ch) {
 #pragma unroll
         for (int pc = 0; pc < PIECES; ++pc) dma_piece(ch, ch, pc);
         dma_w(ch, ch);
     }
-#if DLSA_CYC_FLAGS
-    unsigned long long* const flagL = reinterpret_cast<unsigned long long*>(lds + CYC_NST * BUF);
-    unsigned long long* const flagD = flagL + 4;
-    if (tid < 8) flagL[tid] = 0ull;
-    __syncthreads();
-    auto tag_of = [](int c) { return (unsigned)(((c >> 2) + 1) & 255); };
-    auto post = [&](unsigned long long* f, int stage, int c) {
-        if (lane == 0) reinterpret_cast<volatile unsigned char*>(f + stage)[wave] = (unsigned char)tag_of(c);
-    };
-    auto await = [&](unsigned long long* f, int stage, int c) {
-        const unsigned long long want = 0x0101010101010101ull * tag_of(c);
-        while (__builtin_amdgcn_readfirstlane((int)(*reinterpret_cast<volatile unsigned long long*>(f + stage) != want)))
-            __builtin_amdgcn_s_sleep(1);
-    };
     asm volatile("s_waitcnt vmcnt(%0)" ::"n"(2 * DMA_PER_CHUNK) : "memory");
-    post(flagL, 0, 0);
-    await(flagL, 0, 0);
-#else
-    asm volatile("s_waitcnt vmcnt(%0)" ::"n"(DLSA_CYC_PAIR ? 0 : 2 * DMA_PER_CHUNK) : "memory");
     asm volatile("s_barrier" ::: "memory");
-#endif
 
     const int lane_part = ((lane >> 4) * LDP + (lane & 15)) * 8;
     int adA[2][RW], adB[2][NB], adT[2], adW[2];
 #pragma unroll
     for (int sp = 0; sp < 2; ++sp) {
         const int sb = sp * 2 * BUF * 8;
-        adA[sp][0] = sb + lane_part + 128 * i0;
-        adA[sp][1] = sb + lane_part + 128 * (i0 + 1);
+#pragma unroll
+        for (int r = 0; r < RW; ++r) adA[sp][r] = sb + lane_part + 128 * (i0 + r);
 #pragma unroll
         for (int j = 0; j < NB; ++j) adB[sp][j] = sb + lane_part + 128 * ((i0 + d0 + j) % CYC_NT);
         adT[sp] = sb + ((lane >> 4) * LDP + CYC_C0 + (lane & 3)) * 8;
         adW[sp] = sb + (KC * LDP + (lane >> 4)) * 8;
+    }
+    if constexpr (RW == 1) {
+#pragma unroll
+        for (int sp = 0; sp < 2; ++sp) {
+            asm volatile("" : "+v"(adA[sp][0]), "+v"(adT[sp]), "+v"(adW[sp]));
+#pragma unroll
+            for (int j = 0; j < NB; ++j) asm volatile("" : "+v"(adB[sp][j]));
+        }
     }
     const char* ldsb = (const char*)lds;
     struct Frag { double fa[RW], fb[NB], bt[GA], wv; };
@@ -159,152 +144,104 @@
         }
         f.wv = HASW ? ld(adW[sp], ((ST & 1) * BUF + ks * 4) * 8) : 1.0;
     };
-    auto kstep = [&](const Frag& f, int chunk_dma, int buf_dma, bool issue) {
-        double aw[RW];
-#pragma unroll
-        for (int r = 0; r < RW; ++r) aw[r] = HASW ? f.fa[r] * f.wv : f.fa[r];
-        cyc_row<0>(aw[0], f.fb[0], f.fb[1], f.fb[2], f.fb[3], f.fb[4], f.fb[5], f.fb[6], f.fb[7]);
-        if (issue) {
-#pragma unroll
-            for (int k = 0; k < PPR; ++k) dma_piece(chunk_dma, buf_dma, k);
-        }
-        if (G > 0 || two_rows)
-            cyc_row<1>(aw[1], f.fb[1], f.fb[2], f.fb[3], f.fb[4], f.fb[5], f.fb[6], f.fb[7], f.fb[8]);
-        if (issue) {
-#pragma unroll
-            for (int k = 0; k < PPR; ++k) dma_piece(chunk_dma, buf_dma, PPR + k);
-            dma_w(chunk_dma, buf_dma);
-        }
-        if constexpr (G > 0) {
-            if (tails) cyc_tail_a<RW, G>(aw, f.bt);
-        }
+    const bool last_row_runs = G > 0 || full_rows;
+    auto chunk_barrier = [&]() {
+        asm volatile("s_waitcnt vmcnt(%0)" ::"n"(DMA_PER_CHUNK) : "memory");
+        asm volatile("s_barrier" ::: "memory");
     };
 
-    Frag fr0, fr1;
-    load_frags(0, 0, fr0);
-    if (DLSA_CYC_PRIO == 1 && db) __builtin_amdgcn_s_setprio(1);
-    if (DLSA_CYC_PRIO == 2 && !db) __builtin_amdgcn_s_setprio(1);
-#if DLSA_CYC_FLAGS
-    for (int c4 = 0; c4 < nchunks; c4 += 4) {
-#pragma unroll
-        for (int u = 0; u < 4; ++u) {
-            const int c = c4 + u;
-            load_frags(u, 1, fr1);
-            if (c > 0) post(flagD, (u + 3) & 3, c - 1);
+    if constexpr (RW == 2) {
+        auto kstep = [&](const Frag& f, int chunk_dma, int buf_dma, bool issue) {
+            double aw[RW];
+#pragma unroll
+            for (int r = 0; r < RW; ++r) aw[r] = HASW ? f.fa[r] * f.wv : f.fa[r];
+            cyc_row<0>(aw[0], f.fb[0], f.fb[1], f.fb[2], f.fb[3], f.fb[4], f.fb[5], f.fb[6], f.fb[7]);
+            if (issue) {
+#pragma unroll
+                for (int k = 0; k < PPR; ++k) dma_piece(chunk_dma, buf_dma, k);
+            }
+            if (last_row_runs)
+                cyc_row<1>(aw[1], f.fb[1], f.fb[2], f.fb[3], f.fb[4], f.fb[5], f.fb[6], f.fb[7], f.fb[8]);
+            if (issue) {
+#pragma unroll
+                for (int k = 0; k < PPR; ++k) dma_piece(chunk_dma, buf_dma, PPR + k);
+                dma_w(chunk_dma, buf_dma);
+            }
+            if constexpr (G > 0) {
+                if (tails) cyc_tail_a<RW, G>(aw, f.bt);
+            }
+        };
+
+        Frag fr0, fr1;
+        load_frags(0, 0, fr0);
+        for (int c4 = 0; c4 < nchunks; c4 += 4) {
+#pragma unroll
+            for (int u = 0; u < 4; ++u) {
+                load_frags(u, 1, fr1);
+                __builtin_amdgcn_sched_barrier(0);
+#if DLSA_CYC_SPLIT
+                {
+                    double aw[RW];
+#pragma unroll
+                    for (int r = 0; r < RW; ++r) aw[r] = HASW ? fr0.fa[r] * fr0.wv : fr0.fa[r];
+                    cyc_row<0>(aw[0], fr0.fb[0], fr0.fb[1], fr0.fb[2], fr0.fb[3], fr0.fb[4], fr0.fb[5], fr0.fb[6], fr0.fb[7]);
+                    __builtin_amdgcn_sched_barrier(0);
+                    if (db) chunk_barrier();
+                    if (last_row_runs)
+                        cyc_row<1>(aw[1], fr0.fb[1], fr0.fb[2], fr0.fb[3], fr0.fb[4], fr0.fb[5], fr0.fb[6], fr0.fb[7], fr0.fb[8]);
+                    if constexpr (G > 0) {
+                        if (tails) cyc_tail_a<RW, G>(aw, fr0.bt);
+                    }
+                    __builtin_amdgcn_sched_barrier(0);
+                    if (!db) chunk_barrier();
+                }
+#else
+                kstep(fr0, 0, 0, false);
+                __builtin_amdgcn_sched_barrier(0);
+                chunk_barrier();
+#endif
+                load_frags((u + 1) & 3, 0, fr0);
+                __builtin_amdgcn_sched_barrier(0);
+                kstep(fr1, c4 + u + 3, (u + 3) & 3, true);
+                __builtin_amdgcn_sched_barrier(0);
+            }
+        }
+    } else {
+        const int bq = slot == 0 ? CYC_BAR_Q[0] : slot == 1 ? CYC_BAR_Q[1] : slot == 2 ? CYC_BAR_Q[2] : CYC_BAR_Q[3];
+        auto kstep1 = [&](const Frag& f, int q0) {
+            double aw[1] = {HASW ? f.fa[0] * f.wv : f.fa[0]};
+            if (last_row_runs) cyc_half<0, 0>(aw[0], f.fb[0], f.fb[1], f.fb[2], f.fb[3]);
             __builtin_amdgcn_sched_barrier(0);
-            {
-                double aw[RW];
-#pragma unroll
-                for (int r = 0; r < RW; ++r) aw[r] = HASW ? fr0.fa[r] * fr0.wv : fr0.fa[r];
-                cyc_row<0>(aw[0], fr0.fb[0], fr0.fb[1], fr0.fb[2], fr0.fb[3], fr0.fb[4], fr0.fb[5], fr0.fb[6], fr0.fb[7]);
-                __builtin_amdgcn_sched_barrier(0);
-                asm volatile("s_waitcnt vmcnt(%0)" ::"n"(DMA_PER_CHUNK) : "memory");
-                post(flagL, (u + 1) & 3, c + 1);
-                __builtin_amdgcn_sched_barrier(0);
-                if (G > 0 || two_rows)
-                    cyc_row<1>(aw[1], fr0.fb[1], fr0.fb[2], fr0.fb[3], fr0.fb[4], fr0.fb[5], fr0.fb[6], fr0.fb[7], fr0.fb[8]);
-                if constexpr (G > 0) {
-                    if (tails) cyc_tail_a<RW, G>(aw, fr0.bt);
-                }
-                __builtin_amdgcn_sched_barrier(0);
-            }
-            await(flagL, (u + 1) & 3, c + 1);
-            load_frags((u + 1) & 3, 0, fr0);
+            if (bq == q0 + 1) chunk_barrier();
+            if (last_row_runs) cyc_half<0, 1>(aw[0], f.fb[4], f.fb[5], f.fb[6], f.fb[7]);
+            if constexpr (G > 0) {
+                if (tails) cyc_tail_a<1, G>(aw, f.bt);
+            }
             __builtin_amdgcn_sched_barrier(0);
-            if (c > 0) await(flagD, (u + 3) & 3, c - 1);
-            __builtin_amdgcn_sched_barrier(0);
-            kstep(fr1, c + 3, (u + 3) & 3, true);
-            __builtin_amdgcn_sched_barrier(0);
-        }
-    }
-#elif DLSA_CYC_PAIR
-    for (int c4 = 0; c4 < nchunks; c4 += 4) {
-#pragma unroll
-        for (int u = 0; u < 4; u += 2) {
-            const int c = c4 + u;
-            load_frags(u, 1, fr1);
-            __builtin_amdgcn_sched_barrier(0);
-            kstep(fr0, c + 2, (u + 2) & 3, true);
-            __builtin_amdgcn_sched_barrier(0);
-            load_frags(u + 1, 0, fr0);
-            __builtin_amdgcn_sched_barrier(0);
-            kstep(fr1, c + 3, (u + 3) & 3, true);
-            __builtin_amdgcn_sched_barrier(0);
-            load_frags(u + 1, 1, fr1);
-            __builtin_amdgcn_sched_barrier(0);
-            kstep(fr0, 0, 0, false);
-            __builtin_amdgcn_sched_barrier(0);
-            {
-                double aw[RW];
-#pragma unroll
-                for (int r = 0; r < RW; ++r) aw[r] = HASW ? fr1.fa[r] * fr1.wv : fr1.fa[r];
-                cyc_row<0>(aw[0], fr1.fb[0], fr1.fb[1], fr1.fb[2], fr1.fb[3], fr1.fb[4], fr1.fb[5], fr1.fb[6], fr1.fb[7]);
-                __builtin_amdgcn_sched_barrier(0);
-                if (db) {
-                    asm volatile("s_waitcnt vmcnt(0)" ::: "memory");
-                    asm volatile("s_barrier" ::: "memory");
-                }
-                if (G > 0 || two_rows)
-                    cyc_row<1>(aw[1], fr1.fb[1], fr1.fb[2], fr1.fb[3], fr1.fb[4], fr1.fb[5], fr1.fb[6], fr1.fb[7], fr1.fb[8]);
-                if constexpr (G > 0) {
-                    if (tails) cyc_tail_a<RW, G>(aw, fr1.bt);
-                }
-                __builtin_amdgcn_sched_barrier(0);
-                if (!db) {
-                    asm volatile("s_waitcnt vmcnt(0)" ::: "memory");
-                    asm volatile("s_barrier" ::: "memory");
-                }
-            }
-            load_frags((u + 2) & 3, 0, fr0);
-            __builtin_amdgcn_sched_barrier(0);
-        }
-    }
-#else
-    for (int c4 = 0; c4 < nchunks; c4 += 4) {
-#pragma unroll
-        for (int u = 0; u < 4; ++u) {
-            load_frags(u, 1, fr1);
-            __builtin_amdgcn_sched_barrier(0);
-#if DLSA_CYC_SPLIT
-            {
-                double aw[RW];
-#pragma unroll
-                for (int r = 0; r < RW; ++r) aw[r] = HASW ? fr0.fa[r] * fr0.wv : fr0.fa[r];
-                cyc_row<0>(aw[0], fr0.fb[0], fr0.fb[1], fr0.fb[2], fr0.fb[3], fr0.fb[4], fr0.fb[5], fr0.fb[6], fr0.fb[7]);
-                __builtin_amdgcn_sched_barrier(0);
-                if (db) {
-                    asm volatile("s_waitcnt vmcnt(%0)" ::"n"(DMA_PER_CHUNK) : "memory");
-                    asm volatile("s_barrier" ::: "memory");
-                }
-                if (G > 0 || two_rows)
-                    cyc_row<1>(aw[1], fr0.fb[1], fr0.fb[2], fr0.fb[3], fr0.fb[4], fr0.fb[5], fr0.fb[6], fr0.fb[7], fr0.fb[8]);
-                if constexpr (G > 0) {
-                    if (tails) cyc_tail_a<RW, G>(aw, fr0.bt);
-                }
-                __builtin_amdgcn_sched_barrier(0);
-                if (!db) {
-                    asm volatile("s_waitcnt vmcnt(%0)" ::"n"(DMA_PER_CHUNK) : "memory");
-                    asm volatile("s_barrier" ::: "memory");
-                }
-            }
-#else
-            kstep(fr0, 0, 0, false);
-            __builtin_amdgcn_sched_barrier(0);
-            asm volatile("s_waitcnt vmcnt(%0)" ::"n"(DMA_PER_CHUNK) : "memory");
-            asm volatile("s_barrier" ::: "memory");
-#endif
-            load_frags((u + 1) & 3, 0, fr0);
-            __builtin_amdgcn_sched_barrier(0);
-            kstep(fr1, c4 + u + 3, (u + 3) & 3, true);
-            __builtin_amdgcn_sched_barrier(0);
-        }
-    }
-#endif
+            if (bq == q0 + 2) chunk_barrier();
+        };
+        Frag fr;
+        load_frags(0, 0, fr);
+        for (int c4 = 0; c4 < nchunks; c4 += 4) {
+#pragma unroll
+            for (int u = 0; u < 4; ++u) {
+                kstep1(fr, 0);
+                load_frags(u, 1, fr);
+                __builtin_amdgcn_sched_barrier(0);
+                kstep1(fr, 2);
+#pragma unroll
+                for (int k = 0; k < PPR; ++k) dma_piece(c4 + u + 3, (u + 3) & 3, k);
+                dma_w(c4 + u + 3, (u + 3) & 3);
+                load_frags((u + 1) & 3, 0, fr);
+                __builtin_amdgcn_sched_barrier(0);
+            }
+        }
+    }
     asm volatile("s_waitcnt vmcnt(0)" ::: "memory");
     asm volatile("s_nop 15\n\ts_nop 15" ::: "memory");
 
     double* __restrict__ P = a.partial + (int64_t)slab * CYC_PP * CYC_PP;
-    const int nt_rows = two_rows ? 2 : 1;
+    const int nt_rows = full_rows ? RW : RW - 1;
     cyc_for_tiles<0, 8 * RW>([&](int k, double (&v)[4]) {
         const int r = k >> 3, cdist = k & 7;
         if (r < nt_rows) {
@@ -318,13 +255,23 @@
         }
     });
     if constexpr (G > 0) {
-        if (tails) cyc_for_tails<0, RW * G>([&](int idx, double v) {
+        if (tails) cyc_for_tails<RW, 0, RW * G>([&](int idx, double v) {
             const int s = idx / G, g = idx - s * G;
             const int row = 16 * (i0 + s) + 4 * ((lane & 15) >> 2) + (lane >> 4), col = CYC_C0 + 4 * g + (lane & 3);
             P[(int64_t)row * CYC_PP + col] = v;
         });
     }
     if (probe && lane == 0) *a.clk = __builtin_readcyclecounter() - t_begin;
+}
+
+template <bool HASW, int G>
+__global__ __launch_bounds__(1024 / cyc_rw(G), cyc_rw(G)) void gram_cyclic_kernel(CycArgs a) {
+    cyc_body<HASW, G, cyc_rw(G)>(a);
+}
+
+template <bool HASW, int G>
+__global__ __launch_bounds__(512, 2) void gram_cyclic_rw2_kernel(CycArgs a) {
+    cyc_body<HASW, G, 2>(a);
 }
 
 static int cyc_slabs(int64_t n, int64_t& rows_per_slab) {
@@ -362,19 +309,23 @@
         set_error("gram: workspace %zu bytes needed (256-aligned), got %zu", need, ws_bytes);
         return DLSA_ERR_WORKSPACE;
     }
-    const int g = a.p <= CYC_C0 ? 0 : (a.p - CYC_C0 + 3) / 4;
-    const size_t shm = (size_t)CYC_NST * CYC_BUF * 8 + (DLSA_CYC_FLAGS ? 64 : 0);
+    const int g = a.p <= CYC_C0 ? 0 : std::min((a.p - CYC_C0 + 3) / 4, 3);
+    const size_t shm = (size_t)CYC_NST * CYC_BUF * 8;
     const int blocks = a.nslab * CYC_GROUP;
-#define DLSA_LAUNCH_CYC(HW, GV) do { \
-        DLSA_HIP_CHECK(hipFuncSetAttribute(reinterpret_cast<const void*>(gram_cyclic_kernel<HW, GV>), \
+    const char* knob = kernel_knob("DLSA_GRAM_DBG");
+    const bool twin = knob && (atoi(knob) & 16) && cyc_rw(g) != 2;
+#define DLSA_LAUNCH_CYC(KERNEL, THREADS, HW, GV) do { \
+        DLSA_HIP_CHECK(hipFuncSetAttribute(reinterpret_cast<const void*>(KERNEL<HW, GV>), \
                                            hipFuncAttributeMaxDynamicSharedMemorySize, (int)shm)); \
-        hipLaunchKernelGGL((gram_cyclic_kernel<HW, GV>), dim3(blocks), dim3(512), shm, stream, a); } while (0)
+        hipLaunchKernelGGL((KERNEL<HW, GV>), dim3(blocks), dim3(THREADS), shm, stream, a); } while (0)
 #define DLSA_LAUNCH_CYC_G(HW) do { switch (g) { \
-        case 0: DLSA_LAUNCH_CYC(HW, 0); break; case 1: DLSA_LAUNCH_CYC(HW, 1); break; \
-        case 2: DLSA_LAUNCH_CYC(HW, 2); break; default: DLSA_LAUNCH_CYC(HW, 3); break; } } while (0)
+        case 0: if (twin) DLSA_LAUNCH_CYC(gram_cyclic_rw2_kernel, 512, HW, 0); else DLSA_LAUNCH_CYC(gram_cyclic_kernel, 1024 / cyc_rw(0), HW, 0); break; \
+        case 1: if (twin) DLSA_LAUNCH_CYC(gram_cyclic_rw2_kernel, 512, HW, 1); else DLSA_LAUNCH_CYC(gram_cyclic_kernel, 1024 / cyc_rw(1), HW, 1); break; \
+        case 2: if (twin) DLSA_LAUNCH_CYC(gram_cyclic_rw2_kernel, 512, HW, 2); else DLSA_LAUNCH_CYC(gram_cyclic_kernel, 1024 / cyc_rw(2), HW, 2); break; \
+        default: if (twin) DLSA_LAUNCH_CYC(gram_cyclic_rw2_kernel, 512, HW, 3); else DLSA_LAUNCH_CYC(gram_cyclic_kernel, 1024 / cyc_rw(3), HW, 3); break; } } while (0)
     if (w) DLSA_LAUNCH_CYC_G(true);
     else DLSA_LAUNCH_CYC_G(false);
-    note_gram_kernel(a.clk, stream, "gram_cyclic_kernel<%s,%d>", w ? "true" : "false", g > 3 ? 3 : g);
+    note_gram_kernel(a.clk, stream, twin ? "gram_cyclic_rw2_kernel<%s,%d>" : "gram_cyclic_kernel<%s,%d>", w ? "true" : "false", g);
 #undef DLSA_LAUNCH_CYC_G
 #undef DLSA_LAUNCH_CYC
     DLSA_HIP_CHECK(hipGetLastError());
diff --git a/dlsa_amd/csrc/gram_cyclic_asm.inc b/dlsa_amd/csrc/gram_cyclic_asm.inc
--- a/dlsa_amd/csrc/gram_cyclic_asm.inc
+++ b/dlsa_amd/csrc/gram_cyclic_asm.inc
@@ -1,9 +1,9 @@
 template <int NREG> __device__ __forceinline__ void cyc_acc_zero();
+template <> __device__ __forceinline__ void cyc_acc_zero<64>() {
+    asm volatile("v_accvgpr_write_b32 a0, 0\n\tv_accvgpr_write_b32 a1, 0\n\tv_accvgpr_write_b32 a2, 0\n\tv_accvgpr_write_b32 a3, 0\n\tv_accvgpr_write_b32 a4, 0\n\tv_accvgpr_write_b32 a5, 0\n\tv_accvgpr_write_b32 a6, 0\n\tv_accvgpr_write_b32 a7, 0\n\tv_accvgpr_write_b32 a8, 0\n\tv_accvgpr_write_b32 a9, 0\n\tv_accvgpr_write_b32 a10, 0\n\tv_accvgpr_write_b32 a11, 0\n\tv_accvgpr_write_b32 a12, 0\n\tv_accvgpr_write_b32 a13, 0\n\tv_accvgpr_write_b32 a14, 0\n\tv_accvgpr_write_b32 a15, 0\n\tv_accvgpr_write_b32 a16, 0\n\tv_accvgpr_write_b32 a17, 0\n\tv_accvgpr_write_b32 a18, 0\n\tv_accvgpr_write_b32 a19, 0\n\tv_accvgpr_write_b32 a20, 0\n\tv_accvgpr_write_b32 a21, 0\n\tv_accvgpr_write_b32 a22, 0\n\tv_accvgpr_write_b32 a23, 0\n\tv_accvgpr_write_b32 a24, 0\n\tv_accvgpr_write_b32 a25, 0\n\tv_accvgpr_write_b32 a26, 0\n\tv_accvgpr_write_b32 a27, 0\n\tv_accvgpr_write_b32 a28, 0\n\tv_accvgpr_write_b32 a29, 0\n\tv_accvgpr_write_b32 a30, 0\n\tv_accvgpr_write_b32 a31, 0\n\tv_accvgpr_write_b32 a32, 0\n\tv_accvgpr_write_b32 a33, 0\n\tv_accvgpr_write_b32 a34, 0\n\tv_accvgpr_write_b32 a35, 0\n\tv_accvgpr_write_b32 a36, 0\n\tv_accvgpr_write_b32 a37, 0\n\tv_accvgpr_write_b32 a38, 0\n\tv_accvgpr_write_b32 a39, 0\n\tv_accvgpr_write_b32 a40, 0\n\tv_accvgpr_write_b32 a41, 0\n\tv_accvgpr_write_b32 a42, 0\n\tv_accvgpr_write_b32 a43, 0\n\tv_accvgpr_write_b32 a44, 0\n\tv_accvgpr_write_b32 a45, 0\n\tv_accvgpr_write_b32 a46, 0\n\tv_accvgpr_write_b32 a47, 0\n\tv_accvgpr_write_b32 a48, 0\n\tv_accvgpr_write_b32 a49, 0\n\tv_accvgpr_write_b32 a50, 0\n\tv_accvgpr_write_b32 a51, 0\n\tv_accvgpr_write_b32 a52, 0\n\tv_accvgpr_write_b32 a53, 0\n\tv_accvgpr_write_b32 a54, 0\n\tv_accvgpr_write_b32 a55, 0\n\tv_accvgpr_write_b32 a56, 0\n\tv_accvgpr_write_b32 a57, 0\n\tv_accvgpr_write_b32 a58, 0\n\tv_accvgpr_write_b32 a59, 0\n\tv_accvgpr_write_b32 a60, 0\n\tv_accvgpr_write_b32 a61, 0\n\tv_accvgpr_write_b32 a62, 0\n\tv_accvgpr_write_b32 a63, 0" ::: "a0", "a1", "a2", "a3", "a4", "a5", "a6", "a7", "a8", "a9", "a10", "a11", "a12", "a13", "a14", "a15", "a16", "a17", "a18", "a19", "a20", "a21", "a22", "a23", "a24", "a25", "a26", "a27", "a28", "a29", "a30", "a31", "a32", "a33", "a34", "a35", "a36", "a37", "a38", "a39", "a40", "a41", "a42", "a43", "a44", "a45", "a46", "a47", "a48", "a49", "a50", "a51", "a52", "a53", "a54", "a55", "a56", "a57", "a58", "a59", "a60", "a61", "a62", "a63");
+}
 template <> __device__ __forceinline__ void cyc_acc_zero<128>() {
     asm volatile("v_accvgpr_write_b32 a0, 0\n\tv_accvgpr_write_b32 a1, 0\n\tv_accvgpr_write_b32 a2, 0\n\tv_accvgpr_write_b32 a3, 0\n\tv_accvgpr_write_b32 a4, 0\n\tv_accvgpr_write_b32 a5, 0\n\tv_accvgpr_write_b32 a6, 0\n\tv_accvgpr_write_b32 a7, 0\n\tv_accvgpr_write_b32 a8, 0\n\tv_accvgpr_write_b32 a9, 0\n\tv_accvgpr_write_b32 a10, 0\n\tv_accvgpr_write_b32 a11, 0\n\tv_accvgpr_write_b32 a12, 0\n\tv_accvgpr_write_b32 a13, 0\n\tv_accvgpr_write_b32 a14, 0\n\tv_accvgpr_write_b32 a15, 0\n\tv_accvgpr_write_b32 a16, 0\n\tv_accvgpr_write_b32 a17, 0\n\tv_accvgpr_write_b32 a18, 0\n\tv_accvgpr_write_b32 a19, 0\n\tv_accvgpr_write_b32 a20, 0\n\tv_accvgpr_write_b32 a21, 0\n\tv_accvgpr_write_b32 a22, 0\n\tv_accvgpr_write_b32 a23, 0\n\tv_accvgpr_write_b32 a24, 0\n\tv_accvgpr_write_b32 a25, 0\n\tv_accvgpr_write_b32 a26, 0\n\tv_accvgpr_write_b32 a27, 0\n\tv_accvgpr_write_b32 a28, 0\n\tv_accvgpr_write_b32 a29, 0\n\tv_accvgpr_write_b32 a30, 0\n\tv_accvgpr_write_b32 a31, 0\n\tv_accvgpr_write_b32 a32, 0\n\tv_accvgpr_write_b32 a33, 0\n\tv_accvgpr_write_b32 a34, 0\n\tv_accvgpr_write_b32 a35, 0\n\tv_accvgpr_write_b32 a36, 0\n\tv_accvgpr_write_b32 a37, 0\n\tv_accvgpr_write_b32 a38, 0\n\tv_accvgpr_write_b32 a39, 0\n\tv_accvgpr_write_b32 a40, 0\n\tv_accvgpr_write_b32 a41, 0\n\tv_accvgpr_write_b32 a42, 0\n\tv_accvgpr_write_b32 a43, 0\n\tv_accvgpr_write_b32 a44, 0\n\tv_accvgpr_write_b32 a45, 0\n\tv_accvgpr_write_b32 a46, 0\n\tv_accvgpr_write_b32 a47, 0\n\tv_accvgpr_write_b32 a48, 0\n\tv_accvgpr_write_b32 a49, 0\n\tv_accvgpr_write_b32 a50, 0\n\tv_accvgpr_write_b32 a51, 0\n\tv_accvgpr_write_b32 a52, 0\n\tv_accvgpr_write_b32 a53, 0\n\tv_accvgpr_write_b32 a54, 0\n\tv_accvgpr_write_b32 a55, 0\n\tv_accvgpr_write_b32 a56, 0\n\tv_accvgpr_write_b32 a57, 0\n\tv_accvgpr_write_b32 a58, 0\n\tv_accvgpr_write_b32 a59, 0\n\tv_accvgpr_write_b32 a60, 0\n\tv_accvgpr_write_b32 a61, 0\n\tv_accvgpr_write_b32 a62, 0\n\tv_accvgpr_write_b32 a63, 0\n\tv_accvgpr_write_b32 a64, 0\n\tv_accvgpr_write_b32 a65, 0\n\tv_accvgpr_write_b32 a66, 0\n\tv_accvgpr_write_b32 a67, 0\n\tv_accvgpr_write_b32 a68, 0\n\tv_accvgpr_write_b32 a69, 0\n\tv_accvgpr_write_b32 a70, 0\n\tv_accvgpr_write_b32 a71, 0\n\tv_accvgpr_write_b32 a72, 0\n\tv_accvgpr_write_b32 a73, 0\n\tv_accvgpr_write_b32 a74, 0\n\tv_accvgpr_write_b32 a75, 0\n\tv_accvgpr_write_b32 a76, 0\n\tv_accvgpr_write_b32 a77, 0\n\tv_accvgpr_write_b32 a78, 0\n\tv_accvgpr_write_b32 a79, 0\n\tv_accvgpr_write_b32 a80, 0\n\tv_accvgpr_write_b32 a81, 0\n\tv_accvgpr_write_b32 a82, 0\n\tv_accvgpr_write_b32 a83, 0\n\tv_accvgpr_write_b32 a84, 0\n\tv_accvgpr_write_b32 a85, 0\n\tv_accvgpr_write_b32 a86, 0\n\tv_accvgpr_write_b32 a87, 0\n\tv_accvgpr_write_b32 a88, 0\n\tv_accvgpr_write_b32 a89, 0\n\tv_accvgpr_write_b32 a90, 0\n\tv_accvgpr_write_b32 a91, 0\n\tv_accvgpr_write_b32 a92, 0\n\tv_accvgpr_write_b32 a93, 0\n\tv_accvgpr_write_b32 a94, 0\n\tv_accvgpr_write_b32 a95, 0\n\tv_accvgpr_write_b32 a96, 0\n\tv_accvgpr_write_b32 a97, 0\n\tv_accvgpr_write_b32 a98, 0\n\tv_accvgpr_write_b32 a99, 0\n\tv_accvgpr_write_b32 a100, 0\n\tv_accvgpr_write_b32 a101, 0\n\tv_accvgpr_write_b32 a102, 0\n\tv_accvgpr_write_b32 a103, 0\n\tv_accvgpr_write_b32 a104, 0\n\tv_accvgpr_write_b32 a105, 0\n\tv_accvgpr_write_b32 a106, 0\n\tv_accvgpr_write_b32 a107, 0\n\tv_accvgpr_write_b32 a108, 0\n\tv_accvgpr_write_b32 a109, 0\n\tv_accvgpr_write_b32 a110, 0\n\tv_accvgpr_write_b32 a111, 0\n\tv_accvgpr_write_b32 a112, 0\n\tv_accvgpr_write_b32 a113, 0\n\tv_accvgpr_write_b32 a114, 0\n\tv_accvgpr_write_b32 a115, 0\n\tv_accvgpr_write_b32 a116, 0\n\tv_accvgpr_write_b32 a117, 0\n\tv_accvgpr_write_b32 a118, 0\n\tv_accvgpr_write_b32 a119, 0\n\tv_accvgpr_write_b32 a120, 0\n\tv_accvgpr_write_b32 a121, 0\n\tv_accvgpr_write_b32 a122, 0\n\tv_accvgpr_write_b32 a123, 0\n\tv_accvgpr_write_b32 a124, 0\n\tv_accvgpr_write_b32 a125, 0\n\tv_accvgpr_write_b32 a126, 0\n\tv_accvgpr_write_b32 a127, 0" ::: "a0", "a1", "a2", "a3", "a4", "a5", "a6", "a7", "a8", "a9", "a10", "a11", "a12", "a13", "a14", "a15", "a16", "a17", "a18", "a19", "a20", "a21", "a22", "a23", "a24", "a25", "a26", "a27", "a28", "a29", "a30", "a31", "a32", "a33", "a34", "a35", "a36", "a37", "a38", "a39", "a40", "a41", "a42", "a43", "a44", "a45", "a46", "a47", "a48", "a49", "a50", "a51", "a52", "a53", "a54", "a55", "a56", "a57", "a58", "a59", "a60", "a61", "a62", "a63", "a64", "a65", "a66", "a67", "a68", "a69", "a70", "a71", "a72", "a73", "a74", "a75", "a76", "a77", "a78", "a79", "a80", "a81", "a82", "a83", "a84", "a85", "a86", "a87", "a88", "a89", "a90", "a91", "a92", "a93", "a94", "a95", "a96", "a97", "a98", "a99", "a100", "a101", "a102", "a103", "a104", "a105", "a106", "a107", "a108", "a109", "a110", "a111", "a112", "a113", "a114", "a115", "a116", "a117", "a118", "a119", "a120", "a121", "a122", "a123", "a124", "a125", "a126", "a127");
-}
-template <> __device__ __forceinline__ void cyc_acc_zero<256>() {
-    asm volatile("v_accvgpr_write_b32 a0, 0\n\tv_accvgpr_write_b32 a1, 0\n\tv_accvgpr_write_b32 a2, 0\n\tv_accvgpr_write_b32 a3, 0\n\tv_accvgpr_write_b32 a4, 0\n\tv_accvgpr_write_b32 a5, 0\n\tv_accvgpr_write_b32 a6, 0\n\tv_accvgpr_write_b32 a7, 0\n\tv_accvgpr_write_b32 a8, 0\n\tv_accvgpr_write_b32 a9, 0\n\tv_accvgpr_write_b32 a10, 0\n\tv_accvgpr_write_b32 a11, 0\n\tv_accvgpr_write_b32 a12, 0\n\tv_accvgpr_write_b32 a13, 0\n\tv_accvgpr_write_b32 a14, 0\n\tv_accvgpr_write_b32 a15, 0\n\tv_accvgpr_write_b32 a16, 0\n\tv_accvgpr_write_b32 a17, 0\n\tv_accvgpr_write_b32 a18, 0\n\tv_accvgpr_write_b32 a19, 0\n\tv_accvgpr_write_b32 a20, 0\n\tv_accvgpr_write_b32 a21, 0\n\tv_accvgpr_write_b32 a22, 0\n\tv_accvgpr_write_b32 a23, 0\n\tv_accvgpr_write_b32 a24, 0\n\tv_accvgpr_write_b32 a25, 0\n\tv_accvgpr_write_b32 a26, 0\n\tv_accvgpr_write_b32 a27, 0\n\tv_accvgpr_write_b32 a28, 0\n\tv_accvgpr_write_b32 a29, 0\n\tv_accvgpr_write_b32 a30, 0\n\tv_accvgpr_write_b32 a31, 0\n\tv_accvgpr_write_b32 a32, 0\n\tv_accvgpr_write_b32 a33, 0\n\tv_accvgpr_write_b32 a34, 0\n\tv_accvgpr_write_b32 a35, 0\n\tv_accvgpr_write_b32 a36, 0\n\tv_accvgpr_write_b32 a37, 0\n\tv_accvgpr_write_b32 a38, 0\n\tv_accvgpr_write_b32 a39, 0\n\tv_accvgpr_write_b32 a40, 0\n\tv_accvgpr_write_b32 a41, 0\n\tv_accvgpr_write_b32 a42, 0\n\tv_accvgpr_write_b32 a43, 0\n\tv_accvgpr_write_b32 a44, 0\n\tv_accvgpr_write_b32 a45, 0\n\tv_accvgpr_write_b32 a46, 0\n\tv_accvgpr_write_b32 a47, 0\n\tv_accvgpr_write_b32 a48, 0\n\tv_accvgpr_write_b32 a49, 0\n\tv_accvgpr_write_b32 a50, 0\n\tv_accvgpr_write_b32 a51, 0\n\tv_accvgpr_write_b32 a52, 0\n\tv_accvgpr_write_b32 a53, 0\n\tv_accvgpr_write_b32 a54, 0\n\tv_accvgpr_write_b32 a55, 0\n\tv_accvgpr_write_b32 a56, 0\n\tv_accvgpr_write_b32 a57, 0\n\tv_accvgpr_write_b32 a58, 0\n\tv_accvgpr_write_b32 a59, 0\n\tv_accvgpr_write_b32 a60, 0\n\tv_accvgpr_write_b32 a61, 0\n\tv_accvgpr_write_b32 a62, 0\n\tv_accvgpr_write_b32 a63, 0\n\tv_accvgpr_write_b32 a64, 0\n\tv_accvgpr_write_b32 a65, 0\n\tv_accvgpr_write_b32 a66, 0\n\tv_accvgpr_write_b32 a67, 0\n\tv_accvgpr_write_b32 a68, 0\n\tv_accvgpr_write_b32 a69, 0\n\tv_accvgpr_write_b32 a70, 0\n\tv_accvgpr_write_b32 a71, 0\n\tv_accvgpr_write_b32 a72, 0\n\tv_accvgpr_write_b32 a73, 0\n\tv_accvgpr_write_b32 a74, 0\n\tv_accvgpr_write_b32 a75, 0\n\tv_accvgpr_write_b32 a76, 0\n\tv_accvgpr_write_b32 a77, 0\n\tv_accvgpr_write_b32 a78, 0\n\tv_accvgpr_write_b32 a79, 0\n\tv_accvgpr_write_b32 a80, 0\n\tv_accvgpr_write_b32 a81, 0\n\tv_accvgpr_write_b32 a82, 0\n\tv_accvgpr_write_b32 a83, 0\n\tv_accvgpr_write_b32 a84, 0\n\tv_accvgpr_write_b32 a85, 0\n\tv_accvgpr_write_b32 a86, 0\n\tv_accvgpr_write_b32 a87, 0\n\tv_accvgpr_write_b32 a88, 0\n\tv_accvgpr_write_b32 a89, 0\n\tv_accvgpr_write_b32 a90, 0\n\tv_accvgpr_write_b32 a91, 0\n\tv_accvgpr_write_b32 a92, 0\n\tv_accvgpr_write_b32 a93, 0\n\tv_accvgpr_write_b32 a94, 0\n\tv_accvgpr_write_b32 a95, 0\n\tv_accvgpr_write_b32 a96, 0\n\tv_accvgpr_write_b32 a97, 0\n\tv_accvgpr_write_b32 a98, 0\n\tv_accvgpr_write_b32 a99, 0\n\tv_accvgpr_write_b32 a100, 0\n\tv_accvgpr_write_b32 a101, 0\n\tv_accvgpr_write_b32 a102, 0\n\tv_accvgpr_write_b32 a103, 0\n\tv_accvgpr_write_b32 a104, 0\n\tv_accvgpr_write_b32 a105, 0\n\tv_accvgpr_write_b32 a106, 0\n\tv_accvgpr_write_b32 a107, 0\n\tv_accvgpr_write_b32 a108, 0\n\tv_accvgpr_write_b32 a109, 0\n\tv_accvgpr_write_b32 a110, 0\n\tv_accvgpr_write_b32 a111, 0\n\tv_accvgpr_write_b32 a112, 0\n\tv_accvgpr_write_b32 a113, 0\n\tv_accvgpr_write_b32 a114, 0\n\tv_accvgpr_write_b32 a115, 0\n\tv_accvgpr_write_b32 a116, 0\n\tv_accvgpr_write_b32 a117, 0\n\tv_accvgpr_write_b32 a118, 0\n\tv_accvgpr_write_b32 a119, 0\n\tv_accvgpr_write_b32 a120, 0\n\tv_accvgpr_write_b32 a121, 0\n\tv_accvgpr_write_b32 a122, 0\n\tv_accvgpr_write_b32 a123, 0\n\tv_accvgpr_write_b32 a124, 0\n\tv_accvgpr_write_b32 a125, 0\n\tv_accvgpr_write_b32 a126, 0\n\tv_accvgpr_write_b32 a127, 0\n\tv_accvgpr_write_b32 a128, 0\n\tv_accvgpr_write_b32 a129, 0\n\tv_accvgpr_write_b32 a130, 0\n\tv_accvgpr_write_b32 a131, 0\n\tv_accvgpr_write_b32 a132, 0\n\tv_accvgpr_write_b32 a133, 0\n\tv_accvgpr_write_b32 a134, 0\n\tv_accvgpr_write_b32 a135, 0\n\tv_accvgpr_write_b32 a136, 0\n\tv_accvgpr_write_b32 a137, 0\n\tv_accvgpr_write_b32 a138, 0\n\tv_accvgpr_write_b32 a139, 0\n\tv_accvgpr_write_b32 a140, 0\n\tv_accvgpr_write_b32 a141, 0\n\tv_accvgpr_write_b32 a142, 0\n\tv_accvgpr_write_b32 a143, 0\n\tv_accvgpr_write_b32 a144, 0\n\tv_accvgpr_write_b32 a145, 0\n\tv_accvgpr_write_b32 a146, 0\n\tv_accvgpr_write_b32 a147, 0\n\tv_accvgpr_write_b32 a148, 0\n\tv_accvgpr_write_b32 a149, 0\n\tv_accvgpr_write_b32 a150, 0\n\tv_accvgpr_write_b32 a151, 0\n\tv_accvgpr_write_b32 a152, 0\n\tv_accvgpr_write_b32 a153, 0\n\tv_accvgpr_write_b32 a154, 0\n\tv_accvgpr_write_b32 a155, 0\n\tv_accvgpr_write_b32 a156, 0\n\tv_accvgpr_write_b32 a157, 0\n\tv_accvgpr_write_b32 a158, 0\n\tv_accvgpr_write_b32 a159, 0\n\tv_accvgpr_write_b32 a160, 0\n\tv_accvgpr_write_b32 a161, 0\n\tv_accvgpr_write_b32 a162, 0\n\tv_accvgpr_write_b32 a163, 0\n\tv_accvgpr_write_b32 a164, 0\n\tv_accvgpr_write_b32 a165, 0\n\tv_accvgpr_write_b32 a166, 0\n\tv_accvgpr_write_b32 a167, 0\n\tv_accvgpr_write_b32 a168, 0\n\tv_accvgpr_write_b32 a169, 0\n\tv_accvgpr_write_b32 a170, 0\n\tv_accvgpr_write_b32 a171, 0\n\tv_accvgpr_write_b32 a172, 0\n\tv_accvgpr_write_b32 a173, 0\n\tv_accvgpr_write_b32 a174, 0\n\tv_accvgpr_write_b32 a175, 0\n\tv_accvgpr_write_b32 a176, 0\n\tv_accvgpr_write_b32 a177, 0\n\tv_accvgpr_write_b32 a178, 0\n\tv_accvgpr_write_b32 a179, 0\n\tv_accvgpr_write_b32 a180, 0\n\tv_accvgpr_write_b32 a181, 0\n\tv_accvgpr_write_b32 a182, 0\n\tv_accvgpr_write_b32 a183, 0\n\tv_accvgpr_write_b32 a184, 0\n\tv_accvgpr_write_b32 a185, 0\n\tv_accvgpr_write_b32 a186, 0\n\tv_accvgpr_write_b32 a187, 0\n\tv_accvgpr_write_b32 a188, 0\n\tv_accvgpr_write_b32 a189, 0\n\tv_accvgpr_write_b32 a190, 0\n\tv_accvgpr_write_b32 a191, 0\n\tv_accvgpr_write_b32 a192, 0\n\tv_accvgpr_write_b32 a193, 0\n\tv_accvgpr_write_b32 a194, 0\n\tv_accvgpr_write_b32 a195, 0\n\tv_accvgpr_write_b32 a196, 0\n\tv_accvgpr_write_b32 a197, 0\n\tv_accvgpr_write_b32 a198, 0\n\tv_accvgpr_write_b32 a199, 0\n\tv_accvgpr_write_b32 a200, 0\n\tv_accvgpr_write_b32 a201, 0\n\tv_accvgpr_write_b32 a202, 0\n\tv_accvgpr_write_b32 a203, 0\n\tv_accvgpr_write_b32 a204, 0\n\tv_accvgpr_write_b32 a205, 0\n\tv_accvgpr_write_b32 a206, 0\n\tv_accvgpr_write_b32 a207, 0\n\tv_accvgpr_write_b32 a208, 0\n\tv_accvgpr_write_b32 a209, 0\n\tv_accvgpr_write_b32 a210, 0\n\tv_accvgpr_write_b32 a211, 0\n\tv_accvgpr_write_b32 a212, 0\n\tv_accvgpr_write_b32 a213, 0\n\tv_accvgpr_write_b32 a214, 0\n\tv_accvgpr_write_b32 a215, 0\n\tv_accvgpr_write_b32 a216, 0\n\tv_accvgpr_write_b32 a217, 0\n\tv_accvgpr_write_b32 a218, 0\n\tv_accvgpr_write_b32 a219, 0\n\tv_accvgpr_write_b32 a220, 0\n\tv_accvgpr_write_b32 a221, 0\n\tv_accvgpr_write_b32 a222, 0\n\tv_accvgpr_write_b32 a223, 0\n\tv_accvgpr_write_b32 a224, 0\n\tv_accvgpr_write_b32 a225, 0\n\tv_accvgpr_write_b32 a226, 0\n\tv_accvgpr_write_b32 a227, 0\n\tv_accvgpr_write_b32 a228, 0\n\tv_accvgpr_write_b32 a229, 0\n\tv_accvgpr_write_b32 a230, 0\n\tv_accvgpr_write_b32 a231, 0\n\tv_accvgpr_write_b32 a232, 0\n\tv_accvgpr_write_b32 a233, 0\n\tv_accvgpr_write_b32 a234, 0\n\tv_accvgpr_write_b32 a235, 0\n\tv_accvgpr_write_b32 a236, 0\n\tv_accvgpr_write_b32 a237, 0\n\tv_accvgpr_write_b32 a238, 0\n\tv_accvgpr_write_b32 a239, 0\n\tv_accvgpr_write_b32 a240, 0\n\tv_accvgpr_write_b32 a241, 0\n\tv_accvgpr_write_b32 a242, 0\n\tv_accvgpr_write_b32 a243, 0\n\tv_accvgpr_write_b32 a244, 0\n\tv_accvgpr_write_b32 a245, 0\n\tv_accvgpr_write_b32 a246, 0\n\tv_accvgpr_write_b32 a247, 0\n\tv_accvgpr_write_b32 a248, 0\n\tv_accvgpr_write_b32 a249, 0\n\tv_accvgpr_write_b32 a250, 0\n\tv_accvgpr_write_b32 a251, 0\n\tv_accvgpr_write_b32 a252, 0\n\tv_accvgpr_write_b32 a253, 0\n\tv_accvgpr_write_b32 a254, 0\n\tv_accvgpr_write_b32 a255, 0" ::: "a0", "a1", "a2", "a3", "a4", "a5", "a6", "a7", "a8", "a9", "a10", "a11", "a12", "a13", "a14", "a15", "a16", "a17", "a18", "a19", "a20", "a21", "a22", "a23", "a24", "a25", "a26", "a27", "a28", "a29", "a30", "a31", "a32", "a33", "a34", "a35", "a36", "a37", "a38", "a39", "a40", "a41", "a42", "a43", "a44", "a45", "a46", "a47", "a48", "a49", "a50", "a51", "a52", "a53", "a54", "a55", "a56", "a57", "a58", "a59", "a60", "a61", "a62", "a63", "a64", "a65", "a66", "a67", "a68", "a69", "a70", "a71", "a72", "a73", "a74", "a75", "a76", "a77", "a78", "a79", "a80", "a81", "a82", "a83", "a84", "a85", "a86", "a87", "a88", "a89", "a90", "a91", "a92", "a93", "a94", "a95", "a96", "a97", "a98", "a99", "a100", "a101", "a102", "a103", "a104", "a105", "a106", "a107", "a108", "a109", "a110", "a111", "a112", "a113", "a114", "a115", "a116", "a117", "a118", "a119", "a120", "a121", "a122", "a123", "a124", "a125", "a126", "a127", "a128", "a129", "a130", "a131", "a132", "a133", "a134", "a135", "a136", "a137", "a138", "a139", "a140", "a141", "a142", "a143", "a144", "a145", "a146", "a147", "a148", "a149", "a150", "a151", "a152", "a153", "a154", "a155", "a156", "a157", "a158", "a159", "a160", "a161", "a162", "a163", "a164", "a165", "a166", "a167", "a168", "a169", "a170", "a171", "a172", "a173", "a174", "a175", "a176", "a177", "a178", "a179", "a180", "a181", "a182", "a183", "a184", "a185", "a186", "a187", "a188", "a189", "a190", "a191", "a192", "a193", "a194", "a195", "a196", "a197", "a198", "a199", "a200", "a201", "a202", "a203", "a204", "a205", "a206", "a207", "a208", "a209", "a210", "a211", "a212", "a213", "a214", "a215", "a216", "a217", "a218", "a219", "a220", "a221", "a222", "a223", "a224", "a225", "a226", "a227", "a228", "a229", "a230", "a231", "a232", "a233", "a234", "a235", "a236", "a237", "a238", "a239", "a240", "a241", "a242", "a243", "a244", "a245", "a246", "a247", "a248", "a249", "a250", "a251", "a252", "a253", "a254", "a255");
 }
 template <int R> __device__ __forceinline__ void cyc_row(double a, double b0, double b1, double b2, double b3, double b4, double b5, double b6, double b7);
 template <> __device__ __forceinline__ void cyc_row<0>(double a, double b0, double b1, double b2, double b3, double b4, double b5, double b6, double b7) {
@@ -16,51 +16,90 @@
                  :: "v"(a), "v"(b0), "v"(b1), "v"(b2), "v"(b3), "v"(b4), "v"(b5), "v"(b6), "v"(b7)
                  : "a64", "a65", "a66", "a67", "a68", "a69", "a70", "a71", "a72", "a73", "a74", "a75", "a76", "a77", "a78", "a79", "a80", "a81", "a82", "a83", "a84", "a85", "a86", "a87", "a88", "a89", "a90", "a91", "a92", "a93", "a94", "a95", "a96", "a97", "a98", "a99", "a100", "a101", "a102", "a103", "a104", "a105", "a106", "a107", "a108", "a109", "a110", "a111", "a112", "a113", "a114", "a115", "a116", "a117", "a118", "a119", "a120", "a121", "a122", "a123", "a124", "a125", "a126", "a127");
 }
-template <> __device__ __forceinline__ void cyc_row<2>(double a, double b0, double b1, double b2, double b3, double b4, double b5, double b6, double b7) {
-    asm volatile("s_nop 1\n\tv_mfma_f64_16x16x4_f64 a[128:135], %0, %1, a[128:135]\n\tv_mfma_f64_16x16x4_f64 a[136:143], %0, %2, a[136:143]\n\tv_mfma_f64_16x16x4_f64 a[144:151], %0, %3, a[144:151]\n\tv_mfma_f64_16x16x4_f64 a[152:159], %0, %4, a[152:159]\n\tv_mfma_f64_16x16x4_f64 a[160:167], %0, %5, a[160:167]\n\tv_mfma_f64_16x16x4_f64 a[168:175], %0, %6, a[168:175]\n\tv_mfma_f64_16x16x4_f64 a[176:183], %0, %7, a[176:183]\n\tv_mfma_f64_16x16x4_f64 a[184:191], %0, %8, a[184:191]"
-                 :: "v"(a), "v"(b0), "v"(b1), "v"(b2), "v"(b3), "v"(b4), "v"(b5), "v"(b6), "v"(b7)
-                 : "a128", "a129", "a130", "a131", "a132", "a133", "a134", "a135", "a136", "a137", "a138", "a139", "a140", "a141", "a142", "a143", "a144", "a145", "a146", "a147", "a148", "a149", "a150", "a151", "a152", "a153", "a154", "a155", "a156", "a157", "a158", "a159", "a160", "a161", "a162", "a163", "a164", "a165", "a166", "a167", "a168", "a169", "a170", "a171", "a172", "a173", "a174", "a175", "a176", "a177", "a178", "a179", "a180", "a181", "a182", "a183", "a184", "a185", "a186", "a187", "a188", "a189", "a190", "a191");
+template <int R, int H> __device__ __forceinline__ void cyc_half(double a, double b0, double b1, double b2, double b3);
+template <> __device__ __forceinline__ void cyc_half<0, 0>(double a, double b0, double b1, double b2, double b3) {
+    asm volatile("s_nop 1\n\tv_mfma_f64_16x16x4_f64 a[0:7], %0, %1, a[0:7]\n\tv_mfma_f64_16x16x4_f64 a[8:15], %0, %2, a[8:15]\n\tv_mfma_f64_16x16x4_f64 a[16:23], %0, %3, a[16:23]\n\tv_mfma_f64_16x16x4_f64 a[24:31], %0, %4, a[24:31]"
+                 :: "v"(a), "v"(b0), "v"(b1), "v"(b2), "v"(b3)
+                 : "a0", "a1", "a2", "a3", "a4", "a5", "a6", "a7", "a8", "a9", "a10", "a11", "a12", "a13", "a14", "a15", "a16", "a17", "a18", "a19", "a20", "a21", "a22", "a23", "a24", "a25", "a26", "a27", "a28", "a29", "a30", "a31");
 }
-template <> __device__ __forceinline__ void cyc_row<3>(double a, double b0, double b1, double b2, double b3, double b4, double b5, double b6, double b7) {
-    asm volatile("s_nop 1\n\tv_mfma_f64_16x16x4_f64 a[192:199], %0, %1, a[192:199]\n\tv_mfma_f64_16x16x4_f64 a[200:207], %0, %2, a[200:207]\n\tv_mfma_f64_16x16x4_f64 a[208:215], %0, %3, a[208:215]\n\tv_mfma_f64_16x16x4_f64 a[216:223], %0, %4, a[216:223]\n\tv_mfma_f64_16x16x4_f64 a[224:231], %0, %5, a[224:231]\n\tv_mfma_f64_16x16x4_f64 a[232:239], %0, %6, a[232:239]\n\tv_mfma_f64_16x16x4_f64 a[240:247], %0, %7, a[240:247]\n\tv_mfma_f64_16x16x4_f64 a[248:255], %0, %8, a[248:255]"
-                 :: "v"(a), "v"(b0), "v"(b1), "v"(b2), "v"(b3), "v"(b4), "v"(b5), "v"(b6), "v"(b7)
-                 : "a192", "a193", "a194", "a195", "a196", "a197", "a198", "a199", "a200", "a201", "a202", "a203", "a204", "a205", "a206", "a207", "a208", "a209", "a210", "a211", "a212", "a213", "a214", "a215", "a216", "a217", "a218", "a219", "a220", "a221", "a222", "a223", "a224", "a225", "a226", "a227", "a228", "a229", "a230", "a231", "a232", "a233", "a234", "a235", "a236", "a237", "a238", "a239", "a240", "a241", "a242", "a243", "a244", "a245", "a246", "a247", "a248", "a249", "a250", "a251", "a252", "a253", "a254", "a255");
+template <> __device__ __forceinline__ void cyc_half<0, 1>(double a, double b0, double b1, double b2, double b3) {
+    asm volatile("v_mfma_f64_16x16x4_f64 a[32:39], %0, %1, a[32:39]\n\tv_mfma_f64_16x16x4_f64 a[40:47], %0, %2, a[40:47]\n\tv_mfma_f64_16x16x4_f64 a[48:55], %0, %3, a[48:55]\n\tv_mfma_f64_16x16x4_f64 a[56:63], %0, %4, a[56:63]"
+                 :: "v"(a), "v"(b0), "v"(b1), "v"(b2), "v"(b3)
+                 : "a32", "a33", "a34", "a35", "a36", "a37", "a38", "a39", "a40", "a41", "a42", "a43", "a44", "a45", "a46", "a47", "a48", "a49", "a50", "a51", "a52", "a53", "a54", "a55", "a56", "a57", "a58", "a59", "a60", "a61", "a62", "a63");
+}
+template <> __device__ __forceinline__ void cyc_half<1, 0>(double a, double b0, double b1, double b2, double b3) {
+    asm volatile("s_nop 1\n\tv_mfma_f64_16x16x4_f64 a[64:71], %0, %1, a[64:71]\n\tv_mfma_f64_16x16x4_f64 a[72:79], %0, %2, a[72:79]\n\tv_mfma_f64_16x16x4_f64 a[80:87], %0, %3, a[80:87]\n\tv_mfma_f64_16x16x4_f64 a[88:95], %0, %4, a[88:95]"
+                 :: "v"(a), "v"(b0), "v"(b1), "v"(b2), "v"(b3)
+                 : "a64", "a65", "a66", "a67", "a68", "a69", "a70", "a71", "a72", "a73", "a74", "a75", "a76", "a77", "a78", "a79", "a80", "a81", "a82", "a83", "a84", "a85", "a86", "a87", "a88", "a89", "a90", "a91", "a92", "a93", "a94", "a95");
+}
+template <> __device__ __forceinline__ void cyc_half<1, 1>(double a, double b0, double b1, double b2, double b3) {
+    asm volatile("v_mfma_f64_16x16x4_f64 a[96:103], %0, %1, a[96:103]\n\tv_mfma_f64_16x16x4_f64 a[104:111], %0, %2, a[104:111]\n\tv_mfma_f64_16x16x4_f64 a[112:119], %0, %3, a[112:119]\n\tv_mfma_f64_16x16x4_f64 a[120:127], %0, %4, a[120:127]"
+                 :: "v"(a), "v"(b0), "v"(b1), "v"(b2), "v"(b3)
+                 : "a96", "a97", "a98", "a99", "a100", "a101", "a102", "a103", "a104", "a105", "a106", "a107", "a108", "a109", "a110", "a111", "a112", "a113", "a114", "a115", "a116", "a117", "a118", "a119", "a120", "a121", "a122", "a123", "a124", "a125", "a126", "a127");
 }
 template <int TS, int G> __device__ __forceinline__ void cyc_tail_a(const double (&at)[TS], const double (&bt)[G > 0 ? G : 1]);
-template <int N> __device__ __forceinline__ void cyc_tail_zero();
-template <> __device__ __forceinline__ void cyc_tail_zero<4>() {
+template <int TS, int G> __device__ __forceinline__ void cyc_tail_zero();
+template <> __device__ __forceinline__ void cyc_tail_a<1, 0>(const double (&)[1], const double (&)[1]) {}
+template <> __device__ __forceinline__ void cyc_tail_zero<1, 1>() {
+    asm volatile("v_accvgpr_write_b32 a64, 0\n\tv_accvgpr_write_b32 a65, 0" ::: "a64", "a65");
+}
+template <> __device__ __forceinline__ void cyc_tail_a<1, 1>(const double (&at)[1], const double (&bt)[1]) {
+    asm volatile("v_mfma_f64_4x4x4_4b_f64 a[64:65], %0, %1, a[64:65]"
+                 :: "v"(at[0]), "v"(bt[0])
+                 : "a64", "a65");
+}
+template <> __device__ __forceinline__ void cyc_tail_zero<1, 2>() {
+    asm volatile("v_accvgpr_write_b32 a64, 0\n\tv_accvgpr_write_b32 a65, 0\n\tv_accvgpr_write_b32 a66, 0\n\tv_accvgpr_write_b32 a67, 0" ::: "a64", "a65", "a66", "a67");
+}
+template <> __device__ __forceinline__ void cyc_tail_a<1, 2>(const double (&at)[1], const double (&bt)[2]) {
+    asm volatile("v_mfma_f64_4x4x4_4b_f64 a[64:65], %0, %1, a[64:65]\n\tv_mfma_f64_4x4x4_4b_f64 a[66:67], %0, %2, a[66:67]"
+                 :: "v"(at[0]), "v"(bt[0]), "v"(bt[1])
+                 : "a64", "a65", "a66", "a67");
+}
+template <> __device__ __forceinline__ void cyc_tail_zero<1, 3>() {
+    asm volatile("v_accvgpr_write_b32 a64, 0\n\tv_accvgpr_write_b32 a65, 0\n\tv_accvgpr_write_b32 a66, 0\n\tv_accvgpr_write_b32 a67, 0\n\tv_accvgpr_write_b32 a68, 0\n\tv_accvgpr_write_b32 a69, 0" ::: "a64", "a65", "a66", "a67", "a68", "a69");
+}
+template <> __device__ __forceinline__ void cyc_tail_a<1, 3>(const double (&at)[1], const double (&bt)[3]) {
+    asm volatile("v_mfma_f64_4x4x4_4b_f64 a[64:65], %0, %1, a[64:65]\n\tv_mfma_f64_4x4x4_4b_f64 a[66:67], %0, %2, a[66:67]\n\tv_mfma_f64_4x4x4_4b_f64 a[68:69], %0, %3, a[68:69]"
+                 :: "v"(at[0]), "v"(bt[0]), "v"(bt[1]), "v"(bt[2])
+                 : "a64", "a65", "a66", "a67", "a68", "a69");
+}
+template <> __device__ __forceinline__ void cyc_tail_a<2, 0>(const double (&)[2], const double (&)[1]) {}
+template <> __device__ __forceinline__ void cyc_tail_zero<2, 1>() {
     asm volatile("v_accvgpr_write_b32 a128, 0\n\tv_accvgpr_write_b32 a129, 0\n\tv_accvgpr_write_b32 a130, 0\n\tv_accvgpr_write_b32 a131, 0" ::: "a128", "a129", "a130", "a131");
 }
-template <> __device__ __forceinline__ void cyc_tail_zero<8>() {
-    asm volatile("v_accvgpr_write_b32 a128, 0\n\tv_accvgpr_write_b32 a129, 0\n\tv_accvgpr_write_b32 a130, 0\n\tv_accvgpr_write_b32 a131, 0\n\tv_accvgpr_write_b32 a132, 0\n\tv_accvgpr_write_b32 a133, 0\n\tv_accvgpr_write_b32 a134, 0\n\tv_accvgpr_write_b32 a135, 0" ::: "a128", "a129", "a130", "a131", "a132", "a133", "a134", "a135");
-}
-template <> __device__ __forceinline__ void cyc_tail_zero<12>() {
-    asm volatile("v_accvgpr_write_b32 a128, 0\n\tv_accvgpr_write_b32 a129, 0\n\tv_accvgpr_write_b32 a130, 0\n\tv_accvgpr_write_b32 a131, 0\n\tv_accvgpr_write_b32 a132, 0\n\tv_accvgpr_write_b32 a133, 0\n\tv_accvgpr_write_b32 a134, 0\n\tv_accvgpr_write_b32 a135, 0\n\tv_accvgpr_write_b32 a136, 0\n\tv_accvgpr_write_b32 a137, 0\n\tv_accvgpr_write_b32 a138, 0\n\tv_accvgpr_write_b32 a139, 0" ::: "a128", "a129", "a130", "a131", "a132", "a133", "a134", "a135", "a136", "a137", "a138", "a139");
-}
-template <> __device__ __forceinline__ void cyc_tail_a<2, 0>(const double (&)[2], const double (&)[1]) {}
 template <> __device__ __forceinline__ void cyc_tail_a<2, 1>(const double (&at)[2], const double (&bt)[1]) {
     asm volatile("v_mfma_f64_4x4x4_4b_f64 a[128:129], %0, %2, a[128:129]\n\tv_mfma_f64_4x4x4_4b_f64 a[130:131], %1, %2, a[130:131]"
                  :: "v"(at[0]), "v"(at[1]), "v"(bt[0])
                  : "a128", "a129", "a130", "a131");
+}
+template <> __device__ __forceinline__ void cyc_tail_zero<2, 2>() {
+    asm volatile("v_accvgpr_write_b32 a128, 0\n\tv_accvgpr_write_b32 a129, 0\n\tv_accvgpr_write_b32 a130, 0\n\tv_accvgpr_write_b32 a131, 0\n\tv_accvgpr_write_b32 a132, 0\n\tv_accvgpr_write_b32 a133, 0\n\tv_accvgpr_write_b32 a134, 0\n\tv_accvgpr_write_b32 a135, 0" ::: "a128", "a129", "a130", "a131", "a132", "a133", "a134", "a135");
 }
 template <> __device__ __forceinline__ void cyc_tail_a<2, 2>(const double (&at)[2], const double (&bt)[2]) {
     asm volatile("v_mfma_f64_4x4x4_4b_f64 a[128:129], %0, %2, a[128:129]\n\tv_mfma_f64_4x4x4_4b_f64 a[130:131], %0, %3, a[130:131]\n\tv_mfma_f64_4x4x4_4b_f64 a[132:133], %1, %2, a[132:133]\n\tv_mfma_f64_4x4x4_4b_f64 a[134:135], %1, %3, a[134:135]"
                  :: "v"(at[0]), "v"(at[1]), "v"(bt[0]), "v"(bt[1])
                  : "a128", "a129", "a130", "a131", "a132", "a133", "a134", "a135");
 }
+template <> __device__ __forceinline__ void cyc_tail_zero<2, 3>() {
+    asm volatile("v_accvgpr_write_b32 a128, 0\n\tv_accvgpr_write_b32 a129, 0\n\tv_accvgpr_write_b32 a130, 0\n\tv_accvgpr_write_b32 a131, 0\n\tv_accvgpr_write_b32 a132, 0\n\tv_accvgpr_write_b32 a133, 0\n\tv_accvgpr_write_b32 a134, 0\n\tv_accvgpr_write_b32 a135, 0\n\tv_accvgpr_write_b32 a136, 0\n\tv_accvgpr_write_b32 a137, 0\n\tv_accvgpr_write_b32 a138, 0\n\tv_accvgpr_write_b32 a139, 0" ::: "a128", "a129", "a130", "a131", "a132", "a133", "a134", "a135", "a136", "a137", "a138", "a139");
+}
 template <> __device__ __forceinline__ void cyc_tail_a<2, 3>(const double (&at)[2], const double (&bt)[3]) {
     asm volatile("v_mfma_f64_4x4x4_4b_f64 a[128:129], %0, %2, a[128:129]\n\tv_mfma_f64_4x4x4_4b_f64 a[130:131], %0, %3, a[130:131]\n\tv_mfma_f64_4x4x4_4b_f64 a[132:133], %0, %4, a[132:133]\n\tv_mfma_f64_4x4x4_4b_f64 a[134:135], %1, %2, a[134:135]\n\tv_mfma_f64_4x4x4_4b_f64 a[136:137], %1, %3, a[136:137]\n\tv_mfma_f64_4x4x4_4b_f64 a[138:139], %1, %4, a[138:139]"
                  :: "v"(at[0]), "v"(at[1]), "v"(bt[0]), "v"(bt[1]), "v"(bt[2])
                  : "a128", "a129", "a130", "a131", "a132", "a133", "a134", "a135", "a136", "a137", "a138", "a139");
 }
-template <int IDX> __device__ __forceinline__ double cyc_tail_read() {
+template <int TS, int IDX> __device__ __forceinline__ double cyc_tail_read() {
     int lo, hi;
-    if constexpr (IDX == 0) asm volatile("v_accvgpr_read_b32 %0, a128\n\tv_accvgpr_read_b32 %1, a129" : "=v"(lo), "=v"(hi));
-    else if constexpr (IDX == 1) asm volatile("v_accvgpr_read_b32 %0, a130\n\tv_accvgpr_read_b32 %1, a131" : "=v"(lo), "=v"(hi));
-    else if constexpr (IDX == 2) asm volatile("v_accvgpr_read_b32 %0, a132\n\tv_accvgpr_read_b32 %1, a133" : "=v"(lo), "=v"(hi));
-    else if constexpr (IDX == 3) asm volatile("v_accvgpr_read_b32 %0, a134\n\tv_accvgpr_read_b32 %1, a135" : "=v"(lo), "=v"(hi));
-    else if constexpr (IDX == 4) asm volatile("v_accvgpr_read_b32 %0, a136\n\tv_accvgpr_read_b32 %1, a137" : "=v"(lo), "=v"(hi));
-    else if constexpr (IDX == 5) asm volatile("v_accvgpr_read_b32 %0, a138\n\tv_accvgpr_read_b32 %1, a139" : "=v"(lo), "=v"(hi));
+    if constexpr (TS == 1 && IDX == 0) asm volatile("v_accvgpr_read_b32 %0, a64\n\tv_accvgpr_read_b32 %1, a65" : "=v"(lo), "=v"(hi));
+    else if constexpr (TS == 1 && IDX == 1) asm volatile("v_accvgpr_read_b32 %0, a66\n\tv_accvgpr_read_b32 %1, a67" : "=v"(lo), "=v"(hi));
+    else if constexpr (TS == 1 && IDX == 2) asm volatile("v_accvgpr_read_b32 %0, a68\n\tv_accvgpr_read_b32 %1, a69" : "=v"(lo), "=v"(hi));
+    else if constexpr (TS == 2 && IDX == 0) asm volatile("v_accvgpr_read_b32 %0, a128\n\tv_accvgpr_read_b32 %1, a129" : "=v"(lo), "=v"(hi));
+    else if constexpr (TS == 2 && IDX == 1) asm volatile("v_accvgpr_read_b32 %0, a130\n\tv_accvgpr_read_b32 %1, a131" : "=v"(lo), "=v"(hi));
+    else if constexpr (TS == 2 && IDX == 2) asm volatile("v_accvgpr_read_b32 %0, a132\n\tv_accvgpr_read_b32 %1, a133" : "=v"(lo), "=v"(hi));
+    else if constexpr (TS == 2 && IDX == 3) asm volatile("v_accvgpr_read_b32 %0, a134\n\tv_accvgpr_read_b32 %1, a135" : "=v"(lo), "=v"(hi));
+    else if constexpr (TS == 2 && IDX == 4) asm volatile("v_accvgpr_read_b32 %0, a136\n\tv_accvgpr_read_b32 %1, a137" : "=v"(lo), "=v"(hi));
+    else if constexpr (TS == 2 && IDX == 5) asm volatile("v_accvgpr_read_b32 %0, a138\n\tv_accvgpr_read_b32 %1, a139" : "=v"(lo), "=v"(hi));
     return __hiloint2double(hi, lo);
 }
 template <int T> __device__ __forceinline__ void cyc_tile_read(double (&v)[4]) {
@@ -81,22 +120,6 @@
     else if constexpr (T == 13) asm volatile("v_accvgpr_read_b32 %0, a104\n\tv_accvgpr_read_b32 %1, a105\n\tv_accvgpr_read_b32 %2, a106\n\tv_accvgpr_read_b32 %3, a107\n\tv_accvgpr_read_b32 %4, a108\n\tv_accvgpr_read_b32 %5, a109\n\tv_accvgpr_read_b32 %6, a110\n\tv_accvgpr_read_b32 %7, a111" : "=v"(w0), "=v"(w1), "=v"(w2), "=v"(w3), "=v"(w4), "=v"(w5), "=v"(w6), "=v"(w7));
     else if constexpr (T == 14) asm volatile("v_accvgpr_read_b32 %0, a112\n\tv_accvgpr_read_b32 %1, a113\n\tv_accvgpr_read_b32 %2, a114\n\tv_accvgpr_read_b32 %3, a115\n\tv_accvgpr_read_b32 %4, a116\n\tv_accvgpr_read_b32 %5, a117\n\tv_accvgpr_read_b32 %6, a118\n\tv_accvgpr_read_b32 %7, a119" : "=v"(w0), "=v"(w1), "=v"(w2), "=v"(w3), "=v"(w4), "=v"(w5), "=v"(w6), "=v"(w7));
     else if constexpr (T == 15) asm volatile("v_accvgpr_read_b32 %0, a120\n\tv_accvgpr_read_b32 %1, a121\n\tv_accvgpr_read_b32 %2, a122\n\tv_accvgpr_read_b32 %3, a123\n\tv_accvgpr_read_b32 %4, a124\n\tv_accvgpr_read_b32 %5, a125\n\tv_accvgpr_read_b32 %6, a126\n\tv_accvgpr_read_b32 %7, a127" : "=v"(w0), "=v"(w1), "=v"(w2), "=v"(w3), "=v"(w4), "=v"(w5), "=v"(w6), "=v"(w7));
-    else if constexpr (T == 16) asm volatile("v_accvgpr_read_b32 %0, a128\n\tv_accvgpr_read_b32 %1, a129\n\tv_accvgpr_read_b32 %2, a130\n\tv_accvgpr_read_b32 %3, a131\n\tv_accvgpr_read_b32 %4, a132\n\tv_accvgpr_read_b32 %5, a133\n\tv_accvgpr_read_b32 %6, a134\n\tv_accvgpr_read_b32 %7, a135" : "=v"(w0), "=v"(w1), "=v"(w2), "=v"(w3), "=v"(w4), "=v"(w5), "=v"(w6), "=v"(w7));
-    else if constexpr (T == 17) asm volatile("v_accvgpr_read_b32 %0, a136\n\tv_accvgpr_read_b32 %1, a137\n\tv_accvgpr_read_b32 %2, a138\n\tv_accvgpr_read_b32 %3, a139\n\tv_accvgpr_read_b32 %4, a140\n\tv_accvgpr_read_b32 %5, a141\n\tv_accvgpr_read_b32 %6, a142\n\tv_accvgpr_read_b32 %7, a143" : "=v"(w0), "=v"(w1), "=v"(w2), "=v"(w3), "=v"(w4), "=v"(w5), "=v"(w6), "=v"(w7));
-    else if constexpr (T == 18) asm volatile("v_accvgpr_read_b32 %0, a144\n\tv_accvgpr_read_b32 %1, a145\n\tv_accvgpr_read_b32 %2, a146\n\tv_accvgpr_read_b32 %3, a147\n\tv_accvgpr_read_b32 %4, a148\n\tv_accvgpr_read_b32 %5, a149\n\tv_accvgpr_read_b32 %6, a150\n\tv_accvgpr_read_b32 %7, a151" : "=v"(w0), "=v"(w1), "=v"(w2), "=v"(w3), "=v"(w4), "=v"(w5), "=v"(w6), "=v"(w7));
-    else if constexpr (T == 19) asm volatile("v_accvgpr_read_b32 %0, a152\n\tv_accvgpr_read_b32 %1, a153\n\tv_accvgpr_read_b32 %2, a154\n\tv_accvgpr_read_b32 %3, a155\n\tv_accvgpr_read_b32 %4, a156\n\tv_accvgpr_read_b32 %5, a157\n\tv_accvgpr_read_b32 %6, a158\n\tv_accvgpr_read_b32 %7, a159" : "=v"(w0), "=v"(w1), "=v"(w2), "=v"(w3), "=v"(w4), "=v"(w5), "=v"(w6), "=v"(w7));
-    else if constexpr (T == 20) asm volatile("v_accvgpr_read_b32 %0, a160\n\tv_accvgpr_read_b32 %1, a161\n\tv_accvgpr_read_b32 %2, a162\n\tv_accvgpr_read_b32 %3, a163\n\tv_accvgpr_read_b32 %4, a164\n\tv_accvgpr_read_b32 %5, a165\n\tv_accvgpr_read_b32 %6, a166\n\tv_accvgpr_read_b32 %7, a167" : "=v"(w0), "=v"(w1), "=v"(w2), "=v"(w3), "=v"(w4), "=v"(w5), "=v"(w6), "=v"(w7));
-    else if constexpr (T == 21) asm volatile("v_accvgpr_read_b32 %0, a168\n\tv_accvgpr_read_b32 %1, a169\n\tv_accvgpr_read_b32 %2, a170\n\tv_accvgpr_read_b32 %3, a171\n\tv_accvgpr_read_b32 %4, a172\n\tv_accvgpr_read_b32 %5, a173\n\tv_accvgpr_read_b32 %6, a174\n\tv_accvgpr_read_b32 %7, a175" : "=v"(w0), "=v"(w1), "=v"(w2), "=v"(w3), "=v"(w4), "=v"(w5), "=v"(w6), "=v"(w7));
-    else if constexpr (T == 22) asm volatile("v_accvgpr_read_b32 %0, a176\n\tv_accvgpr_read_b32 %1, a177\n\tv_accvgpr_read_b32 %2, a178\n\tv_accvgpr_read_b32 %3, a179\n\tv_accvgpr_read_b32 %4, a180\n\tv_accvgpr_read_b32 %5, a181\n\tv_accvgpr_read_b32 %6, a182\n\tv_accvgpr_read_b32 %7, a183" : "=v"(w0), "=v"(w1), "=v"(w2), "=v"(w3), "=v"(w4), "=v"(w5), "=v"(w6), "=v"(w7));
-    else if constexpr (T == 23) asm volatile("v_accvgpr_read_b32 %0, a184\n\tv_accvgpr_read_b32 %1, a185\n\tv_accvgpr_read_b32 %2, a186\n\tv_accvgpr_read_b32 %3, a187\n\tv_accvgpr_read_b32 %4, a188\n\tv_accvgpr_read_b32 %5, a189\n\tv_accvgpr_read_b32 %6, a190\n\tv_accvgpr_read_b32 %7, a191" : "=v"(w0), "=v"(w1), "=v"(w2), "=v"(w3), "=v"(w4), "=v"(w5), "=v"(w6), "=v"(w7));
-    else if constexpr (T == 24) asm volatile("v_accvgpr_read_b32 %0, a192\n\tv_accvgpr_read_b32 %1, a193\n\tv_accvgpr_read_b32 %2, a194\n\tv_accvgpr_read_b32 %3, a195\n\tv_accvgpr_read_b32 %4, a196\n\tv_accvgpr_read_b32 %5, a197\n\tv_accvgpr_read_b32 %6, a198\n\tv_accvgpr_read_b32 %7, a199" : "=v"(w0), "=v"(w1), "=v"(w2), "=v"(w3), "=v"(w4), "=v"(w5), "=v"(w6), "=v"(w7));
-    else if constexpr (T == 25) asm volatile("v_accvgpr_read_b32 %0, a200\n\tv_accvgpr_read_b32 %1, a201\n\tv_accvgpr_read_b32 %2, a202\n\tv_accvgpr_read_b32 %3, a203\n\tv_accvgpr_read_b32 %4, a204\n\tv_accvgpr_read_b32 %5, a205\n\tv_accvgpr_read_b32 %6, a206\n\tv_accvgpr_read_b32 %7, a207" : "=v"(w0), "=v"(w1), "=v"(w2), "=v"(w3), "=v"(w4), "=v"(w5), "=v"(w6), "=v"(w7));
-    else if constexpr (T == 26) asm volatile("v_accvgpr_read_b32 %0, a208\n\tv_accvgpr_read_b32 %1, a209\n\tv_accvgpr_read_b32 %2, a210\n\tv_accvgpr_read_b32 %3, a211\n\tv_accvgpr_read_b32 %4, a212\n\tv_accvgpr_read_b32 %5, a213\n\tv_accvgpr_read_b32 %6, a214\n\tv_accvgpr_read_b32 %7, a215" : "=v"(w0), "=v"(w1), "=v"(w2), "=v"(w3), "=v"(w4), "=v"(w5), "=v"(w6), "=v"(w7));
-    else if constexpr (T == 27) asm volatile("v_accvgpr_read_b32 %0, a216\n\tv_accvgpr_read_b32 %1, a217\n\tv_accvgpr_read_b32 %2, a218\n\tv_accvgpr_read_b32 %3, a219\n\tv_accvgpr_read_b32 %4, a220\n\tv_accvgpr_read_b32 %5, a221\n\tv_accvgpr_read_b32 %6, a222\n\tv_accvgpr_read_b32 %7, a223" : "=v"(w0), "=v"(w1), "=v"(w2), "=v"(w3), "=v"(w4), "=v"(w5), "=v"(w6), "=v"(w7));
-    else if constexpr (T == 28) asm volatile("v_accvgpr_read_b32 %0, a224\n\tv_accvgpr_read_b32 %1, a225\n\tv_accvgpr_read_b32 %2, a226\n\tv_accvgpr_read_b32 %3, a227\n\tv_accvgpr_read_b32 %4, a228\n\tv_accvgpr_read_b32 %5, a229\n\tv_accvgpr_read_b32 %6, a230\n\tv_accvgpr_read_b32 %7, a231" : "=v"(w0), "=v"(w1), "=v"(w2), "=v"(w3), "=v"(w4), "=v"(w5), "=v"(w6), "=v"(w7));
-    else if constexpr (T == 29) asm volatile("v_accvgpr_read_b32 %0, a232\n\tv_accvgpr_read_b32 %1, a233\n\tv_accvgpr_read_b32 %2, a234\n\tv_accvgpr_read_b32 %3, a235\n\tv_accvgpr_read_b32 %4, a236\n\tv_accvgpr_read_b32 %5, a237\n\tv_accvgpr_read_b32 %6, a238\n\tv_accvgpr_read_b32 %7, a239" : "=v"(w0), "=v"(w1), "=v"(w2), "=v"(w3), "=v"(w4), "=v"(w5), "=v"(w6), "=v"(w7));
-    else if constexpr (T == 30) asm volatile("v_accvgpr_read_b32 %0, a240\n\tv_accvgpr_read_b32 %1, a241\n\tv_accvgpr_read_b32 %2, a242\n\tv_accvgpr_read_b32 %3, a243\n\tv_accvgpr_read_b32 %4, a244\n\tv_accvgpr_read_b32 %5, a245\n\tv_accvgpr_read_b32 %6, a246\n\tv_accvgpr_read_b32 %7, a247" : "=v"(w0), "=v"(w1), "=v"(w2), "=v"(w3), "=v"(w4), "=v"(w5), "=v"(w6), "=v"(w7));
-    else if constexpr (T == 31) asm volatile("v_accvgpr_read_b32 %0, a248\n\tv_accvgpr_read_b32 %1, a249\n\tv_accvgpr_read_b32 %2, a250\n\tv_accvgpr_read_b32 %3, a251\n\tv_accvgpr_read_b32 %4, a252\n\tv_accvgpr_read_b32 %5, a253\n\tv_accvgpr_read_b32 %6, a254\n\tv_accvgpr_read_b32 %7, a255" : "=v"(w0), "=v"(w1), "=v"(w2), "=v"(w3), "=v"(w4), "=v"(w5), "=v"(w6), "=v"(w7));
     v[0] = __hiloint2double(w1, w0); v[1] = __hiloint2double(w3, w2);
     v[2] = __hiloint2double(w5, w4); v[3] = __hiloint2double(w7, w6);
 }
```
